# csiro-robotics/syropod_highlevel_controller

Hardware: AMD Instinct MI355X
Metric: control-cycles/sec (all legs IK-solved) (higher is better)
Workload: dtype f64

## Files before the change

### syropod_highlevel_controller_amd/csrc/shc_cycle.hpp

```cpp
#pragma once

#include "../../include/shc_batch.h"
#include "shc_leg.hpp"

namespace shc {

enum : int { WS_STARTING = 0, WS_MOVING = 1, WS_STOPPING = 2, WS_STOPPED = 3 };
enum : int { SS_SWING = 0, SS_STANCE = 1, SS_FORCE_STANCE = 2, SS_FORCE_STOP = 3 };
enum : int { PS_POSING = 0, PS_STOP_POSING = 1, PS_POSING_COMPLETE = 2 };
enum : int { PM_NONE = 0, PM_SWING = 1, PM_STANCE = 2, PM_STOP = 3 };

constexpr int LW_ACP = 1 << 2, LW_CFS = 1 << 3, LW_PM_SHIFT = 4, LW_NEG = 1 << 6, LW_IKFAIL = 1 << 7, LW_PHASE_SHIFT = 8,
              LW_PHASE_MASK = 0xFFFFF, LW_ZBV = 1 << 28, LW_ATT = 1 << 29, LW_ROTDEF = 1 << 30,
              LW_TARGROT = int(1u << 31);
constexpr int RW_LACP_SHIFT = 2, RW_LCFS_SHIFT = 6, RW_RTDA = 1 << 10, RW_APS_SHIFT = 11;

constexpr int kMaxAutoPosers = 8;
constexpr int kSwingTable = 64;
enum : unsigned { DIRTY_WALK_PLANE = 1, DIRTY_MANUAL = 2, DIRTY_SWING_ORG = 4, DIRTY_STANCE_ORG = 8,
                  DIRTY_TARG_DIR = 16,
                  DIRTY_LAST = DIRTY_TARG_DIR };
enum : unsigned { RT_MANUAL_LIVE = 1, RT_TOUCHDOWN = 2, RT_EXTERNAL = 4, RT_MANUAL_LEGS = 8, RT_EFFORT_LIVE = 16, RT_SKIP_MARKED = 32, RT_POSE_MARKED = 64 };

enum : unsigned { F_MANUAL = 1, F_AUTO = 2, F_INCL = 4, F_IMU = 8, F_ADM = 16, F_TIPF = 32, F_ODOM = 64, F_DYN = 1u << 31,
                  F_ROT = 1u << 30,
                  F_ROUGH = 1u << 29,
                  F_TALIGN = 1u << 28,
                  F_MLEGS = 1u << 27,
                  F_TERRAIN = F_ROUGH | F_TALIGN | F_MLEGS };
template <int NJ, unsigned F>
constexpr bool rot_enabled() { return (F & F_ROT) != 0 && (NJ > 3 || (F & F_MLEGS) != 0); }

struct CycleParams {
  double dt;
  int32_t period, swing_period, stance_period, stance_end, swing_start, swing_end, stance_start;
  int32_t remap_old_period;
  int32_t swing_iterations;
  int32_t stance_iterations;
  double swing_delta_t;
  double inv_dt;
  double dt_over_swing_dt;
  double stance_dt;
  double stride_scale;
  double swing_height, swing_width, body_clearance;
  double swing_progress_scaler;
  int32_t swing_c_count;
  int32_t swing_c_valid;
  int32_t velocity_input_mode;
  int32_t manual_posing, auto_posing, inclination_posing, imu_posing, admittance_control, dynamic_stiffness, use_joint_effort;
  int32_t clamp_joint_positions, clamp_joint_velocities, force_normal_touchdown;
  int32_t tip_force;
  int32_t debug_skip;
  int32_t odometry;
  int32_t gravity_aligned;
  int32_t rough_terrain;
  int32_t tip_align;
  int32_t gravity_target;
  int32_t joint_control;
  double step_depth;
  double target_dir[3];
  double max_translation[3], max_rotation[3], max_translation_velocity, max_rotation_velocity;
  double pid_p, pid_i, pid_d;
  double adm_m00, adm_m01, adm_m10, adm_m11, adm_g0, adm_g1;
  double force_gain, virtual_stiffness, swing_stiffness_scaler, load_stiffness_scaler;
  double pose_force_gain, pose_swing_height;
  int32_t n_auto_posers, pose_phase_length, pose_sync, auto_pose_reference_leg;
  alignas(16) int32_t ap_start[kMaxAutoPosers];
  int32_t ap_end[kMaxAutoPosers];
  double ap_amp[kMaxAutoPosers][7];
};

template <int L, int NJ>
struct alignas(16) SharedConsts {
  LegConst<NJ> leg[L];
  alignas(16) double limit[9][4];
  double swing_c[kSwingTable];
  alignas(16) CycleParams P;
};

template <int NJ>
struct Fields {
  static constexpr int NJE = (NJ + 1) & ~1;
  static constexpr int Q = 0, QD = NJ, TIP = 2 * NJ, TVEL = TIP + 3, SORG = TVEL + 3, SVEL = SORG + 3, TORG = SVEL + 3,
                       DFLT = TORG + 3, TARG = DFLT + 3, STRD = TARG + 3,
                       CORE_END = STRD + 3,
                       ADM = CORE_END, ADM_END = ADM + 2,
                       TF = ADM_END, TF_END = TF + 4,
                       FORCE_IN = TF_END, EFFORT_IN = FORCE_IN + 4,
                       POSER_TIP = EFFORT_IN + NJE, MODEL_TIP = POSER_TIP + 4, ADM_DELTA = MODEL_TIP + 4,
                       ORG_DIR = ADM_DELTA + 4, CUR_DIR = ORG_DIR + 3,
                       TARG_DIR = CUR_DIR + 3,
                       DES_TIP = TARG_DIR + 4, DES_DIR = DES_TIP + 4,
                       SEQ_ORG = DES_DIR + 4, SEQ_DIR = SEQ_ORG + 4, SEQ_Q0 = SEQ_DIR + 4,
                       STEP_PLANE = SEQ_Q0 + NJE,
                       MEAS_Q = STEP_PLANE + 4, COUNT = MEAS_Q + NJE;
  static_assert(CORE_END % 2 == 0 && SORG % 2 == 0 && COUNT % 2 == 0, "field groups must align to 16-byte planes");
};
SHC_HD int64_t leg_field_index(int f, int64_t slot, int64_t n_slots) { return (int64_t(f >> 1) * n_slots + slot) * 2 + (f & 1); }
struct RobotFields {
  static constexpr int VLIN = 0, VANG = 2, PLANE = 3, PNORM = 6, PLANE_PREV = 9, PNORM_PREV = 12, OWPP = 15, VIN = 22, WIN = 24,
                       CORE_END = 25;
  static constexpr int MPOSE = 25, TVI = 32, RVI = 35, MANUAL_END = 38;
  static constexpr int ABSE = 38, VERR = 41, GYRO = 44, IMU_END = 47;
  static constexpr int IMUQ = 47, IMUQ_END = 51;
  static constexpr int APREV = 51, APREV_END = 55;
  static constexpr int CPOSE = 55, CPOSE_END = 62;
  static constexpr int WPP = 62, WPP_END = 69;
  static constexpr int ODOM = 69, ODOM_END = 73;
  static constexpr int INCL = 73, INCL_END = 75;
  static constexpr int TALIGN = 75, OTALIGN = 82, COUNT = 89;
  static constexpr int I_WORD = 0, I_APOSER = 1, I_POSE_PHASE = 2, I_RESET_MODE = 3, I_COUNT = 4;
};

struct ExtFields {
  static constexpr int T_POSE = 0, T_TRANSFORM = 7, T_CLEARANCE = 14, T_FLAGS = 15,
                       D_POSE = 16, D_TRANSFORM = 23, D_FLAGS = 30,
                       P_POSE = 32, P_TRANSFORM = 39, P_CLEARANCE = 46, P_FLAGS = 47, COUNT = 48;
};

enum : int { LS_WALKING = 0, LS_MANUAL = 1, LS_WALKING_TO_MANUAL = -1, LS_MANUAL_TO_WALKING = -2 };
struct ManualRobot {
  int32_t leg_state[SHC_MAX_LEGS];
  int32_t manual_leg_count, primary_leg, secondary_leg;
  int32_t skip_cycle;
  double primary_velocity[3], secondary_velocity[3];
  double primary_position[3], secondary_position[3];
};

struct DevState {
  double *legd;
  int32_t *legi;
  double *robd;
  int32_t *robi;
  int64_t n_slots, n_rob_pad, n_robots;
  double *ext;
  ManualRobot *manual;
  const double *span;
};

struct SpanTable {
  static constexpr int kPlanes = 14;
  static constexpr int kStride = 2 + 2 * kPlanes;
};
SHC_HD double set_precision3(double v) { return round_to_int(v * 1000.0) / 1000.0; }
SHC_HD double stance_span_change_y(const double *table, int leg, double default_shift_z) {
  const double *t = table + leg * SpanTable::kStride;
  const int n = int(t[0]);
  const double target = set_precision3(default_shift_z);
  int lower = -1, upper = -1;
  for (int k = 0; k < n; ++k) {
    const double h = t[2 + 2 * k];
    if (h > target && (upper < 0 || h < t[2 + 2 * upper])) upper = k;
    if (h <= target && (lower < 0 || h > t[2 + 2 * lower])) lower = k;
  }
  if (lower < 0 || upper < 0) return 0.0;
  const double uh = set_precision3(t[2 + 2 * upper]), lh = set_precision3(t[2 + 2 * lower]);
  const double i = (target - lh) / (uh - lh);
  const double radius = t[3 + 2 * lower] * (1.0 - i) + t[3 + 2 * upper] * i;
  return radius * t[1];
}

#if defined(__HIPCC__)

template <int L, int NJ, unsigned F>
constexpr bool phase_fences() {
#if defined(SHC_FENCE)
  return true;
#else
  constexpr bool exact = (F & (0x80000000u  | 0x40000000u )) == 0;
  constexpr bool octo_tipf = L == 8 && NJ == 5 && (F & 32u ) != 0 && (F & 16u ) == 0;
  return exact && ((NJ == 4 && (L == 4 || L == 8)) || octo_tipf);
#endif
}
#define SHC_PHASE_FENCE() do { if constexpr (phase_fences<L, NJ, F>()) __builtin_amdgcn_sched_barrier(0); } while (0)
#if defined(SHC_RES2_TIMING) && !defined(SHC_RES2_BUSY_ONLY)
__shared__ long long shc_ticks_lds[64];
__shared__ long long shc_acc_lds[64];
#define SHC_TICK(i) do { __builtin_amdgcn_sched_barrier(0); if (blockIdx.x == 1 && (threadIdx.x == 0 || threadIdx.x == 128)) shc_ticks_lds[(threadIdx.x >> 7) * 32 + (i)] = __builtin_readcyclecounter(); __builtin_amdgcn_sched_barrier(0); } while (0)
#else
#define SHC_TICK(i) do {} while (0)
#endif
#ifdef SHC_ABLATE
#define SHC_DBG(P) ((P).debug_skip)
#else
#define SHC_DBG(P) 0
#endif
__device__ __forceinline__ int uni(int v) { return __builtin_amdgcn_readfirstlane(v); }

template <unsigned F>
struct Feat {
  __device__ __forceinline__ static bool manual(const CycleParams &P) { return (F & F_DYN) ? P.manual_posing != 0 : (F & F_MANUAL) != 0; }
  __device__ __forceinline__ static bool autop(const CycleParams &P) { return (F & F_DYN) ? P.auto_posing != 0 : (F & F_AUTO) != 0; }
  __device__ __forceinline__ static bool incl(const CycleParams &P) { return (F & F_DYN) ? P.inclination_posing != 0 : (F & F_INCL) != 0; }
  __device__ __forceinline__ static bool imu(const CycleParams &P) { return (F & F_DYN) ? P.imu_posing != 0 : (F & F_IMU) != 0; }
  __device__ __forceinline__ static bool adm(const CycleParams &P) { return (F & F_DYN) ? P.admittance_control != 0 : (F & F_ADM) != 0; }
  __device__ __forceinline__ static bool tipf(const CycleParams &P) { return (F & F_DYN) ? P.tip_force != 0 : (F & F_TIPF) != 0; }
  __device__ __forceinline__ static bool odom(const CycleParams &P) { return (F & F_DYN) ? P.odometry != 0 : (F & F_ODOM) != 0; }
};

template <int L>
struct Group {
  int base;
  __device__ __forceinline__ int get(int v, int j) const { return __shfl(v, base + j, 64); }
  __device__ __forceinline__ double get(double v, int j) const { return __shfl(v, base + j, 64); }
  __device__ __forceinline__ double sum(double v) const {
    double s = 0.0;
#pragma unroll
    for (int j = 0; j < L; ++j) s += get(v, j);
    return s;
  }
};

template <int RPW>
struct RobTile {
  double *d;
  int32_t *i;
  int grp;
  __device__ __forceinline__ double get(int f) const { return d[f * RPW + grp]; }
  __device__ __forceinline__ V3 get3(int f) const { return V3{d[f * RPW + grp], d[(f + 1) * RPW + grp], d[(f + 2) * RPW + grp]}; }
  __device__ __forceinline__ Quat getq(int f) const {
    return Quat{d[f * RPW + grp], d[(f + 1) * RPW + grp], d[(f + 2) * RPW + grp], d[(f + 3) * RPW + grp]};
  }
  __device__ __forceinline__ Pose getpose(int f) const { return Pose{get3(f), getq(f + 3)}; }
  __device__ __forceinline__ void put(int f, double v) const { d[f * RPW + grp] = v; }
  __device__ __forceinline__ void put3(int f, V3 v) const {
    d[f * RPW + grp] = v.x;
    d[(f + 1) * RPW + grp] = v.y;
    d[(f + 2) * RPW + grp] = v.z;
  }
  __device__ __forceinline__ void putq(int f, Quat q) const {
    d[f * RPW + grp] = q.w;
    d[(f + 1) * RPW + grp] = q.x;
    d[(f + 2) * RPW + grp] = q.y;
    d[(f + 3) * RPW + grp] = q.z;
  }
  __device__ __forceinline__ void putpose(int f, const Pose &p) const {
    put3(f, p.p);
    putq(f + 3, p.r);
  }
  __device__ __forceinline__ int geti(int f) const { return i[f * RPW + grp]; }
  __device__ __forceinline__ void puti(int f, int v) const { i[f * RPW + grp] = v; }
};

template <int NJ>
struct LegRegs {
  static constexpr bool kKeepJacobian = NJ <= 3;
  double q[NJ], qd[NJ];
  double sn[NJ], cs[NJ];
  V3 lin[NJ], pe;
  V3 tip, tvel, targ, strd;
  double adm0, adm1;
  double stiff;
  V3 tf, tipx;
  V3 org_dir, cur_dir, targ_dir;
  int word;
};

enum : int { PK_SORG = 0, PK_SVEL = 3, PK_TORG = 6, PK_DFLT = 9, PK_COUNT = 12 };
#ifndef SHC_PARK_REGS
struct Park {
  double *d;
  int lane;
  __device__ __forceinline__ V3 get3(int f) const { return V3{d[f * 64 + lane], d[(f + 1) * 64 + lane], d[(f + 2) * 64 + lane]}; }
  __device__ __forceinline__ void put3(int f, V3 v) const {
    d[f * 64 + lane] = v.x;
    d[(f + 1) * 64 + lane] = v.y;
    d[(f + 2) * 64 + lane] = v.z;
  }
  __device__ __forceinline__ double at(int k) const { return d[k * 64 + lane]; }
  __device__ __forceinline__ void set(int k, double v) const { d[k * 64 + lane] = v; }
};
#else
struct Park {
  double *d;
  int lane;
  mutable double r[12];
  __device__ __forceinline__ V3 get3(int f) const { return V3{r[f], r[f + 1], r[f + 2]}; }
  __device__ __forceinline__ void put3(int f, V3 v) const { r[f] = v.x, r[f + 1] = v.y, r[f + 2] = v.z; }
  __device__ __forceinline__ double at(int k) const { return r[k]; }
  __device__ __forceinline__ void set(int k, double v) const { r[k] = v; }
};
#endif

__device__ __forceinline__ V3 external_default(const double *ext, int64_t ns, uint32_t slot, V3 terrain_following) {
  if (ext == nullptr) return terrain_following;
  const double2 *X = reinterpret_cast<const double2 *>(ext);
  if ((int(X[(ExtFields::D_FLAGS / 2) * ns + slot].x) & 1) == 0) return terrain_following;
  double v[14];
#pragma unroll
  for (int k = 0; k < 7; ++k) {
    const double2 d = X[(ExtFields::D_POSE / 2 + k) * ns + slot];
    v[2 * k] = d.x, v[2 * k + 1] = d.y;
  }
  return V3{v[0], v[1], v[2]} + rotate(Quat{v[3], v[4], v[5], v[6]}, -V3{v[7], v[8], v[9]});
}

struct LegOut {
  V3 poser_tip, model_tip, adm_delta;
};

__device__ __forceinline__ double swing_progress_of(int word, const CycleParams &P) {
  int pm = (word >> LW_PM_SHIFT) & 3;
  if (pm != PM_SWING) return -1.0;
  int phase = (word >> LW_PHASE_SHIFT) & LW_PHASE_MASK;
  return clampd(double(phase - P.swing_start + 1) / double(P.swing_end - P.swing_start), 0.0, 1.0);
}

__device__ __forceinline__ int bearing_bracket(double y, double x) {
  if (x == 0.0 && y == 0.0) return 0;
  constexpr double kC = 0.99996192306417128874, kS = 0.0087265354983739347;
  double xr = kC * x - kS * y, yr = kS * x + kC * y;
  double ax = fabs(xr), ay = fabs(yr);
  bool upper = yr > 0.0 || (yr == 0.0 && xr > 0.0);
  if (upper) return xr > 0.0 ? (ay < ax ? 0 : 1) : (ay > ax ? 2 : 3);
  return xr < 0.0 ? (ay < ax ? 4 : 5) : (ay > ax ? 6 : 7);
}

template <int NJ>
struct LegInPlanes {
  const double *legd;
  int64_t ns;
  uint32_t slot;
  __device__ __forceinline__ V3 force() const {
    const double2 f01 = reinterpret_cast<const double2 *>(legd)[(Fields<NJ>::FORCE_IN / 2) * ns + slot];
    const double2 f2_ = reinterpret_cast<const double2 *>(legd)[(Fields<NJ>::FORCE_IN / 2 + 1) * ns + slot];
    return V3{f01.x, f01.y, f2_.x};
  }
  __device__ __forceinline__ void effort(double (&e)[NJ]) const {
#pragma unroll
    for (int i = 0; i < NJ; i += 2) {
      const double2 e2 = reinterpret_cast<const double2 *>(legd)[((Fields<NJ>::EFFORT_IN + i) / 2) * ns + slot];
      e[i] = e2.x;
      if (i + 1 < NJ) e[i + 1] = e2.y;
    }
  }
};
struct NoHook {
  __device__ __forceinline__ void operator()() const {}
};

struct UniFlags {
  int clamp_joint_velocities, clamp_joint_positions, swing_c_count;
  int velocity_input_mode, force_normal_touchdown;
};
__device__ __forceinline__ UniFlags load_uni_flags(const CycleParams &P) {
  const int c = P.clamp_joint_velocities, d = P.clamp_joint_positions, e = P.swing_c_count;
  const int f = P.velocity_input_mode, h = P.force_normal_touchdown;
  return UniFlags{uni(c), uni(d), uni(e), uni(f), uni(h)};
}

struct FrontToBack {
  V3 desired_dir;
  bool rot_def;
  int my_leg_state;
  bool plane_prev_changed;
  bool pose_only;
  V3 odom_vel;
  bool odom_run;
  bool joint_moved;
  V3 held_pe, held_dir;
  bool planes_in_sync = false;
  UniFlags uf;
  int limit_bracket = -1;
  double limit_value[4] = {0.0, 0.0, 0.0, 0.0};
};

struct OdomCache {
  double ha = 0.0, sh = 0.0, ch = 1.0;
  bool valid = false;
};
__device__ __forceinline__ void odometry_advance(double &ox, double &oy, double &ow, double &oz, const CycleParams &P, double vx, double vy, double vw,
                                                 OdomCache *cache = nullptr) {
  double sh, ch;
  const double ha = 0.5 * (vw * P.dt);
  if (cache != nullptr && cache->valid && __all(ha == cache->ha)) {
    sh = cache->sh, ch = cache->ch;
  } else {
    if (__all(fabs(ha) <= 0.5)) sincos_joint<false>(ha, &sh, &ch);
    else sincos_joint(ha, &sh, &ch);
    if (cache != nullptr) cache->ha = ha, cache->sh = sh, cache->ch = ch, cache->valid = true;
  }
  {
#pragma clang fp contract(off)
    const double a = vx * P.dt, b = vy * P.dt;
    double ux = -(oz * b), uy = oz * a;
    ux = ux + ux;
    uy = uy + uy;
    const double nx = ox + fma(-oz, uy, fma(ux, ow, a)), ny = oy + fma(oz, ux, fma(uy, ow, b));
    const double nw = fma(ow, ch, -(oz * sh)), nz = fma(ow, sh, oz * ch);
    ox = nx, oy = ny, ow = nw, oz = nz;
  }
}
template <int RPW>
__device__ __forceinline__ void odometry_step(const RobTile<RPW> &rb, const CycleParams &P, double vx, double vy, double vw, OdomCache *cache = nullptr) {
  using R = RobotFields;
  double ox = rb.get(R::ODOM), oy = rb.get(R::ODOM + 1), ow = rb.get(R::ODOM + 2), oz = rb.get(R::ODOM + 3);
  odometry_advance(ox, oy, ow, oz, P, vx, vy, vw, cache);
  rb.put(R::ODOM, ox);
  rb.put(R::ODOM + 1, oy);
  rb.put(R::ODOM + 2, ow);
  rb.put(R::ODOM + 3, oz);
}

template <int L, int NJ>
__device__ __forceinline__ double walk_plane_control_input(const int own_word, const SharedConsts<L, NJ> &C, const CycleParams &P, const Group<L> g,
                                                           const int swing_c_count_u) {
  double c = 0.0;
  bool sel = false;
  if (swing_c_count_u > 0) {
    const int it_own = min(max(((own_word >> LW_PHASE_SHIFT) & LW_PHASE_MASK) - P.swing_start, 0), P.swing_c_count - 1);
    const bool ok_own = ((own_word >> LW_PM_SHIFT) & 3) == PM_SWING && it_own < P.swing_c_valid;
    const unsigned legs_ok = unsigned((__ballot(ok_own) >> g.base) & ((1ull << L) - 1));
    sel = legs_ok != 0;
    const int last = sel ? 31 - __clz(int(legs_ok)) : 0;
    int it_sel = g.get(it_own, last);
    it_sel = sel ? it_sel : 0;
    if (__any(sel)) c = sel ? C.swing_c[it_sel] : 0.0;
  } else {
    double c_own = -1.0;
    const double sp = swing_progress_of(own_word, P) * P.swing_progress_scaler;
    if (sp >= 0 && sp <= 1.0) c_own = smooth_step(sp);
#pragma unroll
    for (int j = 0; j < L; ++j) {
      const double cj = g.get(c_own, j);
      if (cj >= 0.0) {
        c = cj;
        sel = true;
      }
    }
  }
  return sel ? c : -1.0;
}

template <int L, int NJ>
__device__ __forceinline__ double walk_plane_control_candidate(const int own_word, const SharedConsts<L, NJ> &C, const CycleParams &P, const int swing_c_count_u) {
  if (swing_c_count_u > 0) {
    const int it_own = min(max(((own_word >> LW_PHASE_SHIFT) & LW_PHASE_MASK) - P.swing_start, 0), P.swing_c_count - 1);
    const bool ok_own = ((own_word >> LW_PM_SHIFT) & 3) == PM_SWING && it_own < P.swing_c_valid;
    const double c = C.swing_c[it_own];
    return ok_own ? c : -1.0;
  }
  const double sp = swing_progress_of(own_word, P) * P.swing_progress_scaler;
  return (sp >= 0 && sp <= 1.0) ? smooth_step(sp) : -1.0;
}

template <int L>
__device__ __forceinline__ V3 quat_to_euler_zyx_grouped(Quat q, const Group<L> g, const int leg) {
  static_assert(L >= 3, "three lanes per robot");
  double tx = 2.0 * q.x, ty = 2.0 * q.y, tz = 2.0 * q.z;
  double twx = tx * q.w, twy = ty * q.w, twz = tz * q.w;
  double txx = tx * q.x, txy = ty * q.x, txz = tz * q.x;
  double tyy = ty * q.y, tyz = tz * q.y, tzz = tz * q.z;
  double m00 = 1.0 - (tyy + tzz), m01 = txy - twz, m02 = txz + twy;
  double m10 = txy + twz, m11 = 1.0 - (txx + tzz), m12 = tyz - twx;
  double m20 = txz - twy, m21 = tyz + twx, m22 = 1.0 - (txx + tyy);
  const double c2 = sqrt(m22 * m22 + m21 * m21);
  const bool neg = m10 < 0.0 || (m10 == 0.0 && __builtin_signbit(m10) && __builtin_signbit(m00));
  const bool second = leg == 1;
  const double t = atan2(second ? -m20 : m10, second ? (neg ? -c2 : c2) : m00);
  double r0 = g.get(t, 0), r1 = g.get(t, 1);
  if (__builtin_expect(__any((r0 < 0.0) != neg), 0)) r1 = atan2(-m20, r0 < 0.0 ? -c2 : c2);
  if (r0 < 0.0) r0 += kPi;
  double s1, c1;
  sincos_joint(r0, &s1, &c1);
  double r2 = atan2(s1 * m02 - c1 * m12, c1 * m11 - s1 * m01);
  if (fabs(r1) > kPi / 2 || fabs(r2) > kPi / 2) {
    r0 -= kPi;
    if (r1 > kPi / 2.0) r1 = -r1 + kPi;
    else if (r1 < kPi / 2.0) r1 = -r1 - kPi;
    if (r2 > kPi / 2.0) r2 -= kPi;
    else if (r2 < kPi / 2.0) r2 += kPi;
  }
  return V3{r2, r1, r0};
}
template <int L>
__device__ __forceinline__ Quat euler_to_quat_zyx_grouped(V3 e, const Group<L> g, const int leg) {
  static_assert(L >= 3, "three lanes per robot");
  double sn, cs;
  sincos_joint(0.5 * (leg == 0 ? e.x : (leg == 1 ? e.y : e.z)), &sn, &cs);
  const double sx = g.get(sn, 0), cx = g.get(cs, 0), sy = g.get(sn, 1), cy = g.get(cs, 1), sz = g.get(sn, 2), cz = g.get(cs, 2);
  Quat qx{cx, sx, 0, 0}, qy{cy, 0, sy, 0}, qz{cz, 0, 0, sz};
// ... 1139 lines not shown
```

### syropod_highlevel_controller_amd/csrc/shc_cycle_inst.hip

```cpp
#include "shc_cycle_kernel.hpp"
#include "shc_cycle_select.hpp"

#if !defined(SHC_INST_L) || !defined(SHC_INST_NJ) || !defined(SHC_INST_PART)
#error "compile with -DSHC_INST_L=<legs> -DSHC_INST_NJ=<joints> -DSHC_INST_PART=<0|1>"
#endif

#include <cstdio>
#include <cstdlib>
#include <mutex>
#include <set>
#include <tuple>

namespace shc {

static void note_kernel(const char *form, int legs, int joints, unsigned features) {
  static const char *path = std::getenv("SHC_KERNEL_LOG");
  if (!path) return;
  static std::mutex mu;
  static std::set<std::tuple<const char *, unsigned>> seen;
  std::lock_guard<std::mutex> lock(mu);
  if (!seen.insert({form, features}).second) return;
  if (FILE *f = std::fopen(path, "a")) {
    std::fprintf(f, "%s %d %d %u\n", form, legs, joints, features);
    std::fclose(f);
  }
}

template <int L, int NJ, unsigned F>
static void launch_cycle(const CycleLaunch &a) {
  constexpr int RPW = 64 / L;
  constexpr size_t wave_bytes = size_t(RobotFields::COUNT * RPW + PK_COUNT * 64 + (RobotFields::I_COUNT * RPW + 1) / 2) * 8;
#if SHC_INST_PART == 1
  if (a.fit) {
    a.fit->supported = has_resident(F) ? 1 : 0;
    a.fit->batch = has_batch(F) ? 1 : 0;
    a.fit->two_wave = has_two_wave(F) ? 1 : 0;
    a.fit->blocks_per_cu = 0;
    if constexpr (has_resident(F)) {
      int blocks = 0;
      if (hipOccupancyMaxActiveBlocksPerMultiprocessor(&blocks, shc_resident_kernel<L, NJ, F>, 64, wave_bytes) != hipSuccess) blocks = 0;
      a.fit->blocks_per_cu = blocks;
    }
  } else if (a.resident->batch_cycles != 0) {
    if constexpr (has_batch(F)) {
      note_kernel("batch", L, NJ, F);
      shc_batch_kernel<L, NJ, F><<<dim3(a.grid), dim3(a.block), wave_bytes * (a.block / 64), a.stream>>>(a.st, (const SharedConsts<L, NJ> *)a.consts, *a.resident, a.rt_flags);
    }
  } else if (a.block == 256) {
    if constexpr (has_two_wave(F)) {
      note_kernel("resident2", L, NJ, F);
      shc_resident2_kernel<L, NJ, F><<<dim3(a.grid), dim3(256), 2 * wave_bytes + sizeof(Resident2Lds<L, NJ>), a.stream>>>(
          a.st, (const SharedConsts<L, NJ> *)a.consts, *a.resident, a.rt_flags);
    }
  } else {
    if constexpr (has_resident(F)) {
      note_kernel("resident", L, NJ, F);
      shc_resident_kernel<L, NJ, F><<<dim3(a.grid), dim3(64), wave_bytes, a.stream>>>(a.st, (const SharedConsts<L, NJ> *)a.consts, *a.resident, a.rt_flags);
    }
  }
#else
  if constexpr (has_half_kernels(F)) {
    const int64_t waves = int64_t(a.grid) * (a.block / 64);
    if (a.half_steps >= 0 && (a.half_steps > 0 || waves >= 2048)) {
      note_kernel("half", L, NJ, F);
      for (int c = 0; c < a.n_cycles; ++c) {
        shc_cycle_half_kernel<L, NJ, F, ROLE_FRONT><<<dim3(a.grid), dim3(a.block), wave_bytes * (a.block / 64), a.stream>>>(
            a.st, (const SharedConsts<L, NJ> *)a.consts, a.rt_flags, a.wave0);
        shc_cycle_half_kernel<L, NJ, F, ROLE_BACK><<<dim3(a.grid), dim3(a.block), wave_bytes * (a.block / 64), a.stream>>>(
            a.st, (const SharedConsts<L, NJ> *)a.consts, a.rt_flags, a.wave0);
      }
      return;
    }
  }
  note_kernel("cycle", L, NJ, F);
  shc_cycle_kernel<L, NJ, F><<<dim3(a.grid), dim3(a.block), wave_bytes * (a.block / 64), a.stream>>>(a.st, (const SharedConsts<L, NJ> *)a.consts, a.n_cycles,
                                                                                              a.rt_flags, a.wave0);
#endif
}

template <int L, int NJ, unsigned... Fs>
static bool launch_selected(const CycleLaunch &a, FeatureList<Fs...>) {
  const unsigned f = select_features(L, NJ, *a.cp, a.rt_flags, a.generic);
  return ((f == Fs && (launch_cycle<L, NJ, Fs>(a), true)) || ...);
}

#define SHC_CAT3(a, b, c) a##b##_##c
#define SHC_LAUNCHER_NAME(L_, NJ_) SHC_CAT3(shc_launch_cycle_, L_, NJ_)
#define SHC_LOOP_LAUNCHER_NAME(L_, NJ_) SHC_CAT3(shc_launch_loop_, L_, NJ_)
#if SHC_INST_PART == 1
bool SHC_LOOP_LAUNCHER_NAME(SHC_INST_L, SHC_INST_NJ)(const CycleLaunch &a) { return launch_selected<SHC_INST_L, SHC_INST_NJ>(a, KernelTable<SHC_INST_L, SHC_INST_NJ>{}); }
#else
bool SHC_LOOP_LAUNCHER_NAME(SHC_INST_L, SHC_INST_NJ)(const CycleLaunch &a);
bool SHC_LAUNCHER_NAME(SHC_INST_L, SHC_INST_NJ)(const CycleLaunch &a) {
  if (a.fit || a.resident) return SHC_LOOP_LAUNCHER_NAME(SHC_INST_L, SHC_INST_NJ)(a);
  return launch_selected<SHC_INST_L, SHC_INST_NJ>(a, KernelTable<SHC_INST_L, SHC_INST_NJ>{});
}
#endif

}
```

### syropod_highlevel_controller_amd/csrc/shc_cycle_kernel.hpp

```cpp
#pragma once

#include "shc_cycle.hpp"
#include "shc_cycle_launch.hpp"

#include <hip/hip_runtime.h>

namespace shc {

#ifndef SHC_WAVES_PER_SIMD
#define SHC_WAVES_PER_SIMD 2
#endif
#ifndef SHC_ROT_WAVES_PER_SIMD
#define SHC_ROT_WAVES_PER_SIMD 1
#endif
#ifndef SHC_TERRAIN_WAVES_PER_SIMD
#define SHC_TERRAIN_WAVES_PER_SIMD 2
#endif

struct LegPlanes {
  double2 *base;
  int64_t ns;
  uint32_t slot;
  typedef double v2d __attribute__((ext_vector_type(2)));
  __device__ __forceinline__ double2 load(int plane) const { return (base + plane * ns)[slot]; }
  __device__ __forceinline__ void store(int plane, double2 v) const {
    v2d w = {v.x, v.y};
    __builtin_nontemporal_store(w, reinterpret_cast<v2d *>(base + plane * ns + slot));
  }
};

template <int NJ>
struct LegLoad {
  double flat[Fields<NJ>::CORE_END];
  double2 adm, tf0, tf1, stiff, rot0, rot1, rot2, rot3, rot4;
  int word;
};
enum : int { ROLE_ALL = 0, ROLE_FRONT = 1, ROLE_BACK = 2 };
template <int NJ, unsigned F, int ROLE = ROLE_ALL>
__device__ __forceinline__ void load_leg_issue(LegLoad<NJ> &ll, const DevState &st, const CycleParams &P, uint32_t slot) {
  using FD = Fields<NJ>;
  using FT = Feat<F>;
  const LegPlanes ld{reinterpret_cast<double2 *>(st.legd), st.n_slots, slot};
#pragma unroll
  for (int p = 0; p < FD::CORE_END / 2; ++p) {
    if ((ROLE == ROLE_FRONT && p < NJ) || (ROLE == ROLE_BACK && p >= NJ)) {
      ll.flat[2 * p] = ll.flat[2 * p + 1] = 0.0;
      continue;
    }
    double2 v = ld.load(p);
    ll.flat[2 * p] = v.x;
    ll.flat[2 * p + 1] = v.y;
  }
  ll.word = ROLE == ROLE_BACK ? 0 : st.legi[slot];
  ll.adm = ll.tf0 = ll.tf1 = ll.stiff = ll.rot0 = ll.rot1 = ll.rot2 = ll.rot3 = ll.rot4 = double2{0.0, 0.0};
  if (rot_enabled<NJ, F>() && ROLE != ROLE_BACK) {
    ll.rot0 = ld.load(FD::ORG_DIR / 2);
    ll.rot1 = ld.load(FD::ORG_DIR / 2 + 1);
    ll.rot2 = ld.load(FD::ORG_DIR / 2 + 2);
    ll.rot3 = ld.load(FD::ORG_DIR / 2 + 3);
    ll.rot4 = ld.load(FD::ORG_DIR / 2 + 4);
  }
  if (FT::adm(P)) {
    if (ROLE != ROLE_FRONT) ll.adm = ld.load(FD::ADM / 2);
    if (ROLE != ROLE_BACK && P.dynamic_stiffness) ll.stiff = ld.load(FD::ADM_DELTA / 2 + 1);
  }
  if (FT::tipf(P) && ROLE != ROLE_FRONT) {
    ll.tf0 = ld.load(FD::TF / 2);
    ll.tf1 = ld.load(FD::TF / 2 + 1);
  }
}
template <int NJ, int ROLE = ROLE_ALL>
__device__ __forceinline__ void load_leg_finish(LegRegs<NJ> &s, const Park &pk, const LegLoad<NJ> &ll) {
  using FD = Fields<NJ>;
  const double(&flat)[FD::CORE_END] = ll.flat;
  s.word = ll.word;
  static_assert(FD::SVEL == FD::SORG + 3 && FD::TORG == FD::SORG + 6 && FD::DFLT == FD::SORG + 9, "park layout");
  if (ROLE != ROLE_BACK) {
#pragma unroll
    for (int k = 0; k < PK_COUNT; ++k) pk.set(k, flat[FD::SORG + k]);
  }
  s.tip = V3{flat[FD::TIP + 0], flat[FD::TIP + 1], flat[FD::TIP + 2]};
  s.targ = V3{flat[FD::TARG + 0], flat[FD::TARG + 1], flat[FD::TARG + 2]};
  s.strd = V3{flat[FD::STRD + 0], flat[FD::STRD + 1], flat[FD::STRD + 2]};
  s.tvel = V3{flat[FD::TVEL + 0], flat[FD::TVEL + 1], flat[FD::TVEL + 2]};
#pragma unroll
  for (int i = 0; i < NJ; ++i) {
    s.q[i] = flat[FD::Q + i];
    s.qd[i] = flat[FD::QD + i];
  }
  s.adm0 = ll.adm.x;
  s.adm1 = ll.adm.y;
  s.stiff = ll.stiff.y;
  s.tf = V3{ll.tf0.x, ll.tf0.y, ll.tf1.x};
  s.org_dir = V3{ll.rot0.x, ll.rot0.y, ll.rot1.x};
  s.cur_dir = V3{ll.rot1.y, ll.rot2.x, ll.rot2.y};
  s.targ_dir = V3{ll.rot3.x, ll.rot3.y, ll.rot4.x};
}

template <int NJ, unsigned F, int ROLE = ROLE_ALL, bool SPLIT = false>
__device__ __forceinline__ void store_leg(const LegRegs<NJ> &s, const LegOut &out, const Park &pk, const DevState &st, const CycleParams &P,
                                          uint32_t slot, unsigned dirty) {
  using FD = Fields<NJ>;
  using FT = Feat<F>;
  const LegPlanes ld{reinterpret_cast<double2 *>(st.legd), st.n_slots, slot};
  double flat[FD::CORE_END];
#pragma unroll
  for (int i = 0; i < NJ; ++i) {
    flat[FD::Q + i] = s.q[i];
    flat[FD::QD + i] = s.qd[i];
  }
  flat[FD::TIP] = s.tip.x, flat[FD::TIP + 1] = s.tip.y, flat[FD::TIP + 2] = s.tip.z;
  flat[FD::TVEL] = s.tvel.x, flat[FD::TVEL + 1] = s.tvel.y, flat[FD::TVEL + 2] = s.tvel.z;
#pragma unroll
  for (int k = 0; k < PK_COUNT; ++k) flat[FD::SORG + k] = ROLE == ROLE_BACK ? 0.0 : pk.at(k);
  flat[FD::TARG] = s.targ.x, flat[FD::TARG + 1] = s.targ.y, flat[FD::TARG + 2] = s.targ.z;
  flat[FD::STRD] = s.strd.x, flat[FD::STRD + 1] = s.strd.y, flat[FD::STRD + 2] = s.strd.z;
  static_assert(FD::SORG % 2 == 0 && FD::TORG % 2 == 0 && FD::TARG % 2 == 0, "park groups must cover whole planes");
#pragma unroll
  for (int p = 0; p < FD::CORE_END / 2; ++p) {
    const bool swing_org = 2 * p >= FD::SORG && 2 * p < FD::TORG, stance_org = 2 * p >= FD::TORG && 2 * p < FD::TARG;
    if (swing_org && !(dirty & DIRTY_SWING_ORG)) continue;
    if (stance_org && !(dirty & DIRTY_STANCE_ORG)) continue;
    if ((ROLE == ROLE_FRONT && p < NJ) || (ROLE == ROLE_BACK && p >= NJ)) continue;
    ld.store(p, double2{flat[2 * p], flat[2 * p + 1]});
  }
  if (FT::adm(P) && ROLE != ROLE_FRONT && !(SPLIT && ROLE == ROLE_BACK)) {
    ld.store(FD::ADM / 2, double2{s.adm0, s.adm1});
    ld.store(FD::ADM_DELTA / 2, double2{out.adm_delta.x, out.adm_delta.y});
    ld.store(FD::ADM_DELTA / 2 + 1, double2{out.adm_delta.z, s.stiff});
  }
  if (SPLIT && ROLE == ROLE_FRONT && FT::adm(P) && P.dynamic_stiffness) st.legd[leg_field_index(FD::ADM_DELTA + 3, slot, st.n_slots)] = s.stiff;
  if (FT::tipf(P) && ROLE != ROLE_FRONT) {
    ld.store(FD::TF / 2, double2{s.tf.x, s.tf.y});
    ld.store(FD::TF / 2 + 1, double2{s.tf.z, 0.0});
  }
  if (FT::autop(P) && !FT::imu(P) && ROLE != ROLE_BACK) {
    ld.store(FD::POSER_TIP / 2, double2{out.poser_tip.x, out.poser_tip.y});
    ld.store(FD::POSER_TIP / 2 + 1, double2{out.poser_tip.z, 0.0});
  }
  if (rot_enabled<NJ, F>() && ROLE != ROLE_BACK) {
    static_assert(FD::ORG_DIR % 2 == 0 && FD::CUR_DIR == FD::ORG_DIR + 3 && FD::TARG_DIR == FD::ORG_DIR + 6, "tip direction planes");
    ld.store(FD::ORG_DIR / 2, double2{s.org_dir.x, s.org_dir.y});
    ld.store(FD::ORG_DIR / 2 + 1, double2{s.org_dir.z, s.cur_dir.x});
    ld.store(FD::ORG_DIR / 2 + 2, double2{s.cur_dir.y, s.cur_dir.z});
    if (dirty & DIRTY_TARG_DIR) {
      ld.store(FD::ORG_DIR / 2 + 3, double2{s.targ_dir.x, s.targ_dir.y});
      ld.store(FD::ORG_DIR / 2 + 4, double2{s.targ_dir.z, 0.0});
    }
  }
  if (ROLE != ROLE_BACK) st.legi[slot] = s.word;
}

template <int NJ>
__device__ __forceinline__ void store_admittance_early(const LegRegs<NJ> &s, const LegOut &out, const DevState &st, uint32_t slot) {
  using FD = Fields<NJ>;
  const LegPlanes ld{reinterpret_cast<double2 *>(st.legd), st.n_slots, slot};
  ld.store(FD::ADM / 2, double2{s.adm0, s.adm1});
  ld.store(FD::ADM_DELTA / 2, double2{out.adm_delta.x, out.adm_delta.y});
  st.legd[leg_field_index(FD::ADM_DELTA + 2, slot, st.n_slots)] = out.adm_delta.z;
}

template <int RPW, int F0, int F1>
__device__ __forceinline__ void load_rob_fields(double (&reg)[((F1 - F0) * RPW + 63) / 64], const double *gtile, int lane) {
  constexpr int total = (F1 - F0) * RPW;
  constexpr int iters = (total + 63) / 64;
#pragma unroll
  for (int it = 0; it < iters; ++it) {
    int idx = it * 64 + lane;
    reg[it] = idx < total ? gtile[F0 * RPW + idx] : 0.0;
  }
}
template <int RPW, int F0, int F1>
__device__ __forceinline__ void put_rob_fields(const double (&reg)[((F1 - F0) * RPW + 63) / 64], double *tile, int lane) {
  constexpr int total = (F1 - F0) * RPW;
  constexpr int iters = (total + 63) / 64;
#pragma unroll
  for (int it = 0; it < iters; ++it) {
    int idx = it * 64 + lane;
    if (idx < total) tile[F0 * RPW + idx] = reg[it];
  }
}
template <int RPW, int F0, int F1>
__device__ __forceinline__ void store_rob_fields(const double *tile, double *gtile, int lane) {
  constexpr int total = (F1 - F0) * RPW;
  constexpr int iters = (total + 63) / 64;
#pragma unroll
  for (int it = 0; it < iters; ++it) {
    int idx = it * 64 + lane;
    if (idx < total) gtile[F0 * RPW + idx] = tile[F0 * RPW + idx];
  }
}

typedef unsigned long long u64;
__device__ __forceinline__ u64 ld_agent(const u64 *p) { return __hip_atomic_load(p, __ATOMIC_RELAXED, __HIP_MEMORY_SCOPE_AGENT); }
__device__ __forceinline__ void st_agent(u64 *p, u64 v) { __hip_atomic_store(p, v, __ATOMIC_RELAXED, __HIP_MEMORY_SCOPE_AGENT); }
__device__ __forceinline__ u64 ld_sys(const u64 *p) { return __hip_atomic_load(p, __ATOMIC_RELAXED, __HIP_MEMORY_SCOPE_SYSTEM); }
__device__ __forceinline__ void st_sys(u64 *p, u64 v) { __hip_atomic_store(p, v, __ATOMIC_RELAXED, __HIP_MEMORY_SCOPE_SYSTEM); }
__device__ __forceinline__ double ld_agent_f64(const double *p) { return __longlong_as_double((long long)ld_agent(reinterpret_cast<const u64 *>(p))); }
__device__ __forceinline__ u64 uni64(u64 v) {
  const unsigned lo = __builtin_amdgcn_readfirstlane(unsigned(v)), hi = __builtin_amdgcn_readfirstlane(unsigned(v >> 32));
  return (u64(hi) << 32) | lo;
}

template <int NJ>
struct LegInRing {
  const double *force_ptr = nullptr, *effort_ptr = nullptr;
  int64_t force_pair = 0, effort_pair = 0;
  bool effort_prefetched = false;
  double effort_now[NJ] = {};
  bool coherent = true;
  bool force_prefetched = false;
  double force_now[3] = {};
  __device__ __forceinline__ double ld(const double *p) const { return coherent ? ld_agent_f64(p) : *p; }
  __device__ __forceinline__ void prefetch_effort() {
#pragma unroll
    for (int i = 0; i < NJ; ++i) effort_now[i] = ld(effort_ptr + int64_t(i / 2) * effort_pair + (i & 1));
    effort_prefetched = true;
  }
  __device__ __forceinline__ void prefetch_force() {
    force_now[0] = ld(force_ptr), force_now[1] = ld(force_ptr + 1), force_now[2] = ld(force_ptr + force_pair);
    force_prefetched = true;
  }
  __device__ __forceinline__ V3 force() const {
    if (force_prefetched) return V3{force_now[0], force_now[1], force_now[2]};
    return V3{ld(force_ptr), ld(force_ptr + 1), ld(force_ptr + force_pair)};
  }
  __device__ __forceinline__ void effort(double (&e)[NJ]) const {
    if (effort_prefetched) {
#pragma unroll
      for (int i = 0; i < NJ; ++i) e[i] = effort_now[i];
      return;
    }
#pragma unroll
    for (int i = 0; i < NJ; ++i) e[i] = ld(effort_ptr + int64_t(i / 2) * effort_pair + (i & 1));
  }
};
__device__ __forceinline__ const double *bound_array(const ResidentArgs &A, int set, int which) {
  const double *const *row = set == 0 ? A.bound[0] : (set == 1 ? A.bound[1] : (set == 2 ? A.bound[2] : A.bound[3]));
  return which == BND_LIN ? row[BND_LIN] : which == BND_ANG ? row[BND_ANG] : which == BND_IMUQ ? row[BND_IMUQ] : which == BND_IMUW ? row[BND_IMUW]
       : which == BND_FORCE ? row[BND_FORCE] : row[BND_EFFORT];
}
template <int L, int NJ>
__device__ __forceinline__ LegInRing<NJ> leg_inputs_in_force(const ResidentArgs &A, const double *legd, const int src_force, const int src_effort, const int64_t ns,
                                                             const uint32_t slot, const int64_t robot, const int leg, const int64_t row = 0) {
  using FD = Fields<NJ>;
  LegInRing<NJ> in;
  const double *fplanes = src_force < 0 ? legd + int64_t(FD::FORCE_IN / 2) * ns * 2 : A.force + int64_t(src_force) * 2 * ns * 2;
  const double *eplanes = src_effort < 0 ? legd + int64_t(FD::EFFORT_IN / 2) * ns * 2 : A.effort + int64_t(src_effort) * (FD::NJE / 2) * ns * 2;
  in.force_ptr = fplanes + int64_t(slot) * 2, in.force_pair = ns * 2;
  in.effort_ptr = eplanes + int64_t(slot) * 2, in.effort_pair = ns * 2;
  if (src_force <= -2) in.force_ptr = bound_array(A, -2 - src_force, BND_FORCE) + row * A.kstride[BND_FORCE] + (robot * L + leg) * 3, in.force_pair = 2;
  if (src_effort <= -2) in.effort_ptr = bound_array(A, -2 - src_effort, BND_EFFORT) + row * A.kstride[BND_EFFORT] + (robot * L + leg) * NJ, in.effort_pair = 2;
  return in;
}

struct ResidentHeld {
  int src_force = -1, src_effort = -1;
  unsigned seen = 0;
  unsigned cycles = 0;
  bool fault = false;
};

template <int RPW, int NF>
__device__ __forceinline__ void ring_to_tile(const double *rec, double *tile_at, int lane) {
  constexpr int total = NF * RPW;
#pragma unroll
  for (int it = 0; it * 64 < total; ++it) {
    const int i = it * 64 + lane;
    if (i < total) tile_at[i] = ld_agent_f64(rec + i);
  }
}

enum : int { ROBOT_NONE = 0, ROBOT_VEL = 1, ROBOT_POSE = 2, ROBOT_ALL = 3 };
template <int RPW, int ROBOT, bool LEG>
__device__ __forceinline__ void resident_take_inputs(const ResidentArgs &A, const unsigned c, const u64 h0, const u64 h1, const int64_t wave, const int lane,
                                                     double *tile, int32_t *tile_i, unsigned &dirty, ResidentHeld &held, const int64_t n_robots, const int64_t row = 0) {
  using R = RobotFields;
  if (h0 != u64(c) + 1) return;
  const unsigned mask = unsigned(h1) & 0x7fffu;
  held.seen |= mask;
  if (unsigned(h1) & kResidentDirect) {
    const int set = int((h1 >> 16) & 3);
    if (ROBOT != ROBOT_NONE) {
      if ((ROBOT & ROBOT_VEL) && (mask & (1u << RG_VEL))) {
        static_assert(R::WIN == R::VIN + 2, "velocity inputs are contiguous in the tile");
        const double *lin = bound_array(A, set, BND_LIN) + row * A.kstride[BND_LIN], *ang = bound_array(A, set, BND_ANG) + row * A.kstride[BND_ANG];
        const int field = lane / RPW, r = lane - field * RPW;
        const int64_t rob = wave * RPW + r;
        if (lane < 3 * RPW && rob < n_robots) tile[(R::VIN + field) * RPW + r] = field < 2 ? ld_agent_f64(lin + rob * 2 + field) : ld_agent_f64(ang + rob);
      }
      if ((ROBOT & ROBOT_POSE) && (mask & (1u << RG_IMU))) {
        const int64_t rob = wave * RPW + lane;
        if (lane < RPW && rob < n_robots) {
          const double *q = bound_array(A, set, BND_IMUQ) + row * A.kstride[BND_IMUQ] + rob * 4, *w = bound_array(A, set, BND_IMUW) + row * A.kstride[BND_IMUW] + rob * 3;
          const Quat qn = normalized(Quat{ld_agent_f64(q), ld_agent_f64(q + 1), ld_agent_f64(q + 2), ld_agent_f64(q + 3)});
          tile[(R::IMUQ + 0) * RPW + lane] = qn.w, tile[(R::IMUQ + 1) * RPW + lane] = qn.x, tile[(R::IMUQ + 2) * RPW + lane] = qn.y, tile[(R::IMUQ + 3) * RPW + lane] = qn.z;
#pragma unroll
          for (int k = 0; k < 3; ++k) tile[(R::GYRO + k) * RPW + lane] = ld_agent_f64(w + k);
        }
      }
      __builtin_amdgcn_fence(__ATOMIC_RELEASE, "wavefront");
      __builtin_amdgcn_wave_barrier();
    }
    if (LEG) {
      if (mask & (1u << RG_FORCE)) held.src_force = -2 - set;
      if (mask & (1u << RG_EFFORT)) held.src_effort = -2 - set;
    }
    return;
// ... 338 lines not shown
          st_agent(&A.ctl->pad[1], m);
          asm volatile("s_waitcnt vmcnt(0)" ::: "memory");
          st_agent(&A.ctl->pad[2], 1ull);
          st_sys(&A.host->exited, (fault || gave_up) ? u64(RESIDENT_EXIT_FAULT) : why);
        }
      }
      if ((++iter & 1023) == 0 && lane == 0) st_sys(&A.host->heartbeat, iter);
    }
    if (leave) break;
    __builtin_amdgcn_s_sleep(1);
  }
}

template <int L, int NJ, unsigned F, bool RES, int HALF = ROLE_ALL, bool BATCH = false>
__device__ __forceinline__ void cycle_wave(const DevState &st, const SharedConsts<L, NJ> *gc, int n_cycles, unsigned rt_flags, const int64_t wave,
                                           const ResidentArgs *ra) {
  static_assert(HALF == ROLE_ALL || (!RES && (F & (F_DYN | F_TERRAIN | F_MLEGS | F_AUTO)) == 0), "half-step launches: feature-exact kernels without auto posing / terrain paths");
  using R = RobotFields;
  using FT = Feat<F>;
  constexpr int RPW = 64 / L;
  __shared__ SharedConsts<L, NJ> C;
  extern __shared__ double wave_lds[];
  constexpr int kWaveDoubles = R::COUNT * RPW + PK_COUNT * 64 + (R::I_COUNT * RPW + 1) / 2;
  SHC_TICK(0);
  const bool manual_live = (rt_flags & RT_MANUAL_LIVE) != 0;
  const bool touchdown_detection = (rt_flags & RT_TOUCHDOWN) != 0;
  const int lane = threadIdx.x & 63;
  const int wib = threadIdx.x >> 6;
  const int64_t rob0 = wave * RPW;
  const int64_t left = st.n_robots - rob0;
  const int robots_here = left < RPW ? (left < 0 ? 0 : int(left)) : RPW;
  int grp = lane / L;
  const int leg = lane - grp * L;
  const bool live = grp < robots_here;
  if (grp >= robots_here) grp = robots_here > 0 ? robots_here - 1 : 0;
  const uint32_t slot = uint32_t(wave * 64 + grp * L + leg);
  double *const my_lds = wave_lds + wib * kWaveDoubles;
  Park pk{my_lds + R::COUNT * RPW, lane};
  LegRegs<NJ> s;
  const CycleParams &GP = gc->P;
  double *tile = my_lds;
  int32_t *tile_i = reinterpret_cast<int32_t *>(my_lds + R::COUNT * RPW + PK_COUNT * 64);
  double *gtile = st.robd + wave * (R::COUNT * RPW);
  int32_t *gtile_i = st.robi + wave * (R::I_COUNT * RPW);
  LegLoad<NJ> ll;
  double th[NJ];
  const bool any_robot = robots_here > 0;
  double2 hand[4] = {double2{0.0, 0.0}, double2{0.0, 0.0}, double2{0.0, 0.0}, double2{0.0, 0.0}};
  double hpose[7] = {0.0, 0.0, 0.0, 1.0, 0.0, 0.0, 0.0};
  double2 qpl[(NJ + 1) / 2];
  int word_back = 0;
  if (any_robot) {
#pragma unroll
    for (int k = 0; k < NJ; ++k) th[k] = gc->leg[leg].link_th[k];
    load_leg_issue<NJ, F, HALF>(ll, st, GP, slot);
    if constexpr (HALF == ROLE_FRONT) {
#pragma unroll
      for (int p = 0; p < (NJ + 1) / 2; ++p) qpl[p] = reinterpret_cast<const double2 *>(st.legd)[p * st.n_slots + slot];
    }
    if constexpr (HALF == ROLE_BACK) {
      word_back = st.legi[slot];
      using FDh = Fields<NJ>;
      static_assert(FDh::TIP % 2 == 0 && FDh::CUR_DIR == FDh::ORG_DIR + 3 && FDh::ORG_DIR % 2 == 0, "plane layout of the walker tip / tip direction");
      const double2 *planes = reinterpret_cast<const double2 *>(st.legd);
      hand[0] = planes[(FDh::TIP / 2) * st.n_slots + slot];
      hand[1] = planes[(FDh::TIP / 2 + 1) * st.n_slots + slot];
      hand[2] = planes[(FDh::ORG_DIR / 2 + 1) * st.n_slots + slot];
      hand[3] = planes[(FDh::ORG_DIR / 2 + 2) * st.n_slots + slot];
#pragma unroll
      for (int k = 0; k < 7; ++k) hpose[k] = gtile[(R::CPOSE + k) * RPW + grp];
    }
  }
  using SC = SharedConsts<L, NJ>;
  static_assert(sizeof(SC) % 16 == 0 && (offsetof(SC, P) + offsetof(CycleParams, ap_start)) % 16 == 0, "const block is copied in 16-byte words");
  constexpr int n16_all = sizeof(SC) / 16;
  constexpr int n16_core = (offsetof(SC, P) + offsetof(CycleParams, ap_start)) / 16;
  const int n16 = FT::autop(GP) ? n16_all : n16_core;
  constexpr int citers = (n16_all + 63) / 64;
  double2 creg[citers];
  {
    const double2 *src = reinterpret_cast<const double2 *>(gc);
    const int nt = blockDim.x;
#pragma unroll
    for (int it = 0; it < citers; ++it) {
      int i = it * nt + threadIdx.x;
      creg[it] = i < n16 ? src[i] : double2{0.0, 0.0};
    }
  }
  double t_core[(R::CORE_END * RPW + 63) / 64], t_man[((R::MANUAL_END - R::MPOSE) * RPW + 63) / 64],
      t_imu[((R::IMU_END - R::ABSE) * RPW + 63) / 64], t_imuq[((R::IMUQ_END - R::IMUQ) * RPW + 63) / 64],
      t_aprev[((R::APREV_END - R::APREV) * RPW + 63) / 64], t_align[((R::COUNT - R::TALIGN) * RPW + 63) / 64], t_odom[((R::ODOM_END - R::ODOM) * RPW + 63) / 64],
      t_cpose[((R::CPOSE_END - R::CPOSE) * RPW + 63) / 64], t_incl[((R::INCL_END - R::INCL) * RPW + 63) / 64];
  const bool skip_marked = (F & F_MLEGS) != 0 && (rt_flags & RT_SKIP_MARKED) != 0 && (rt_flags & RT_MANUAL_LEGS) != 0;
  const bool pose_marked = (F & F_MLEGS) != 0 && (rt_flags & RT_POSE_MARKED) != 0 && (rt_flags & RT_MANUAL_LEGS) != 0;
  constexpr int int_iters = (R::I_COUNT * RPW + 63) / 64;
  int32_t t_int[int_iters];
  if (any_robot && HALF == ROLE_BACK) {
#pragma unroll
    for (int k = 0; k < NJ; ++k) sincos_joint(th[k] + ll.flat[Fields<NJ>::Q + k], &s.sn[k], &s.cs[k]);
    load_leg_finish<NJ, HALF>(s, pk, ll);
    s.word = word_back;
  }
  if (any_robot && HALF != ROLE_BACK) {
    load_rob_fields<RPW, 0, R::CORE_END>(t_core, gtile, lane);
    if (FT::manual(GP) && manual_live) load_rob_fields<RPW, R::MPOSE, R::MANUAL_END>(t_man, gtile, lane);
    if (FT::imu(GP)) load_rob_fields<RPW, R::ABSE, R::IMU_END>(t_imu, gtile, lane);
    if (FT::imu(GP) || FT::incl(GP) || FT::autop(GP)) load_rob_fields<RPW, R::IMUQ, R::IMUQ_END>(t_imuq, gtile, lane);
    if (FT::incl(GP) && FT::autop(GP)) load_rob_fields<RPW, R::APREV, R::APREV_END>(t_aprev, gtile, lane);
    if (FT::odom(GP)) load_rob_fields<RPW, R::ODOM, R::ODOM_END>(t_odom, gtile, lane);
    if (skip_marked || pose_marked) load_rob_fields<RPW, R::CPOSE, R::CPOSE_END>(t_cpose, gtile, lane);
    if (pose_marked && FT::incl(GP)) load_rob_fields<RPW, R::INCL, R::INCL_END>(t_incl, gtile, lane);
    if ((F & F_TALIGN) != 0 && GP.tip_align) load_rob_fields<RPW, R::TALIGN, R::COUNT>(t_align, gtile, lane);
#pragma unroll
    for (int it = 0; it < int_iters; ++it) t_int[it] = it * 64 + lane < R::I_COUNT * RPW ? gtile_i[it * 64 + lane] : 0;
#pragma unroll
    for (int k = 0; k < NJ; ++k) {
      double qk = ll.flat[Fields<NJ>::Q + k];
      if constexpr (HALF == ROLE_FRONT) qk = (k & 1) ? qpl[k / 2].y : qpl[k / 2].x;
      sincos_joint(th[k] + qk, &s.sn[k], &s.cs[k]);
    }
    load_leg_finish<NJ, HALF>(s, pk, ll);
  }
  {
    double2 *dst = reinterpret_cast<double2 *>(&C);
    const int nt = blockDim.x;
#pragma unroll
    for (int it = 0; it < citers; ++it) {
      int i = it * nt + threadIdx.x;
      if (i < n16) dst[i] = creg[it];
    }
  }
  if (any_robot && HALF != ROLE_BACK) {
    put_rob_fields<RPW, 0, R::CORE_END>(t_core, tile, lane);
    if (FT::manual(GP) && manual_live) put_rob_fields<RPW, R::MPOSE, R::MANUAL_END>(t_man, tile, lane);
    if (FT::imu(GP)) put_rob_fields<RPW, R::ABSE, R::IMU_END>(t_imu, tile, lane);
    if (FT::imu(GP) || FT::incl(GP) || FT::autop(GP)) put_rob_fields<RPW, R::IMUQ, R::IMUQ_END>(t_imuq, tile, lane);
    if (FT::incl(GP) && FT::autop(GP)) put_rob_fields<RPW, R::APREV, R::APREV_END>(t_aprev, tile, lane);
    if (FT::odom(GP)) put_rob_fields<RPW, R::ODOM, R::ODOM_END>(t_odom, tile, lane);
    if (skip_marked || pose_marked) put_rob_fields<RPW, R::CPOSE, R::CPOSE_END>(t_cpose, tile, lane);
    if (pose_marked && FT::incl(GP)) put_rob_fields<RPW, R::INCL, R::INCL_END>(t_incl, tile, lane);
    if ((F & F_TALIGN) != 0 && GP.tip_align) put_rob_fields<RPW, R::TALIGN, R::COUNT>(t_align, tile, lane);
#pragma unroll
    for (int it = 0; it < int_iters; ++it)
      if (it * 64 + lane < R::I_COUNT * RPW) tile_i[it * 64 + lane] = t_int[it];
  }
  SHC_TICK(18);
  __syncthreads();
  SHC_TICK(19);
  if (robots_here == 0) return;
  const CycleParams &P = C.P;
  Group<L> g{grp * L};
  RobTile<RPW> rb{tile, tile_i, grp};
  s.tipx = V3{1, 0, 0};
  constexpr bool rot_on = rot_enabled<NJ, F>();
  if (FT::adm(P) || LegRegs<NJ>::kKeepJacobian || rot_on) {
    Chain<NJ> ch;
    chain_from_sincos<NJ>(C.leg[leg], s.sn, s.cs, ch);
    if (LegRegs<NJ>::kKeepJacobian) {
      jacobian_columns<NJ>(ch, s.lin);
      s.pe = ch.pe;
    }
    if (FT::adm(P) || rot_on) s.tipx = base_rotate(C.leg[leg], ch.xe);
  }
  LegOut out;
  SHC_TICK(1);
  unsigned dirty = 0;
  double *const ext = ((F & F_ROUGH) != 0 && (rt_flags & RT_EXTERNAL) != 0) ? st.ext : nullptr;
  const ManualRobot *const mr = ((F & F_MLEGS) != 0 && (rt_flags & RT_MANUAL_LEGS) != 0 && any_robot) ? st.manual + (rob0 + grp) : nullptr;
  const bool marked = mr != nullptr && mr->skip_cycle != 0;
  const bool skip = (skip_marked && marked) || (pose_marked && !marked);
  const bool pose_only = pose_marked && marked;
  ResidentHeld held;
  if constexpr (RES) {
    resident_loop<L, NJ, F, BATCH>(*ra, st, s, out, C, rb, pk, g, leg, slot, lane, wave, live, tile, tile_i, dirty, manual_live, held, touchdown_detection, ext);
  } else if constexpr (HALF == ROLE_FRONT) {
    FrontToBack fb;
    fb.planes_in_sync = false;
    fb.limit_bracket = -1;
    fb.uf = load_uni_flags(C.P);
    fb.pose_only = false;
    cycle_front<L, NJ, F, (F & F_ADM) == 0>(s, out, C, rb, pk, g, leg, st.legd, st.n_slots, slot, dirty, manual_live, touchdown_detection, ext, mr,
                                            LegInPlanes<NJ>{st.legd, st.n_slots, slot}, fb);
  } else if constexpr (HALF == ROLE_BACK) {
    FrontToBack fb;
    fb.uf = load_uni_flags(C.P);
    fb.pose_only = false;
    fb.joint_moved = false;
    fb.my_leg_state = 0;
    fb.rot_def = (s.word & LW_ROTDEF) != 0;
    {
      const Pose bp{V3{hpose[0], hpose[1], hpose[2]}, Quat{hpose[3], hpose[4], hpose[5], hpose[6]}};
      out.poser_tip = inverse_transform_vector(bp, V3{hand[0].x, hand[0].y, hand[1].x});
      fb.desired_dir = V3{1, 0, 0};
      if (fb.rot_def) fb.desired_dir = rotate(inverse(bp.r), V3{hand[2].y, hand[3].x, hand[3].y});
    }
    out.adm_delta = V3{0.0, 0.0, 0.0};
    if (FT::adm(P)) {
      cycle_admittance<NJ>(s, out, P, LegInPlanes<NJ>{st.legd, st.n_slots, slot});
      if (live && !skip) store_admittance_early<NJ>(s, out, st, slot);
    }
    cycle_back<L, NJ, F>(s, out, C, leg, st.legd, st.n_slots, slot, mr, LegInPlanes<NJ>{st.legd, st.n_slots, slot}, fb);
  } else if (!skip) {
    for (int c = 0; c < n_cycles; ++c)
      cycle<L, NJ, F>(s, out, C, rb, pk, g, leg, st.legd, st.n_slots, slot, dirty, manual_live, touchdown_detection, ext, mr,
                      LegInPlanes<NJ>{st.legd, st.n_slots, slot}, NoHook(), (F & F_ROUGH) != 0 ? st.span : nullptr, pose_only);
    if ((F & F_MLEGS) != 0 && pose_only && FT::autop(P) && !FT::imu(P)) {
      const double2 *planes = reinterpret_cast<const double2 *>(st.legd);
      const double2 a = planes[(Fields<NJ>::POSER_TIP / 2) * st.n_slots + slot], b = planes[(Fields<NJ>::POSER_TIP / 2 + 1) * st.n_slots + slot];
      out.poser_tip = V3{a.x, a.y, b.x};
    }
  }
  {
    unsigned d = 0;
#pragma unroll
    for (unsigned b = 1; b <= DIRTY_LAST; b <<= 1)
      if (__any((dirty & b) != 0)) d |= b;
    dirty = d;
  }
  if (live && !skip) store_leg<NJ, F, HALF, HALF != ROLE_ALL>(s, out, pk, st, P, slot, dirty);
  if constexpr (HALF == ROLE_BACK) {
    if (live) st.legi[slot] = s.word;
    return;
  }
  SHC_TICK(13);
  __builtin_amdgcn_wave_barrier();
  store_rob_fields<RPW, 0, R::PLANE>(tile, gtile, lane);
  if (dirty & DIRTY_WALK_PLANE) store_rob_fields<RPW, R::PLANE, R::VIN>(tile, gtile, lane);
  if (FT::manual(P) && manual_live && (dirty & DIRTY_MANUAL)) store_rob_fields<RPW, R::MPOSE, R::MANUAL_END>(tile, gtile, lane);
  if (FT::imu(P)) store_rob_fields<RPW, R::ABSE, R::GYRO>(tile, gtile, lane);
  if (FT::incl(P) && FT::autop(P)) store_rob_fields<RPW, R::APREV, R::APREV_END>(tile, gtile, lane);
  if ((F & F_MLEGS) != 0 && FT::incl(P) && pose_marked) store_rob_fields<RPW, R::INCL, R::INCL_END>(tile, gtile, lane);
  store_rob_fields<RPW, R::CPOSE, R::CPOSE_END>(tile, gtile, lane);
  if (FT::odom(P)) store_rob_fields<RPW, R::ODOM, R::ODOM_END>(tile, gtile, lane);
  if ((F & F_TALIGN) != 0 && P.tip_align) store_rob_fields<RPW, R::TALIGN, R::COUNT>(tile, gtile, lane);
  static_assert((R::I_POSE_PHASE + 1) * RPW <= 64, "the written-back int fields (word, poser latches, pose phase) fit one wave-wide store");
  if (lane < (R::I_POSE_PHASE + 1) * RPW) gtile_i[lane] = tile_i[lane];
  if constexpr (RES) resident_epilogue<L, NJ, F>(*ra, st, slot, lane, live, tile, tile_i, gtile, gtile_i, held);
  SHC_TICK(14);
}

template <int L, int NJ, unsigned F>
__global__ void __launch_bounds__(256, (F & F_ROT) ? SHC_ROT_WAVES_PER_SIMD : ((F & F_DYN) && (F & F_TERRAIN)) ? SHC_TERRAIN_WAVES_PER_SIMD : SHC_WAVES_PER_SIMD) shc_cycle_kernel(DevState st, const SharedConsts<L, NJ> *gc, int n_cycles,
                                                                                             unsigned rt_flags, int64_t wave0) {
  cycle_wave<L, NJ, F, false>(st, gc, n_cycles, rt_flags, wave0 + ((int64_t(blockIdx.x) * blockDim.x + threadIdx.x) >> 6), nullptr);
}

template <int L, int NJ, unsigned F, int HALF>
__global__ void __launch_bounds__(256, 2) shc_cycle_half_kernel(DevState st, const SharedConsts<L, NJ> *gc, unsigned rt_flags, int64_t wave0) {
  cycle_wave<L, NJ, F, false, HALF>(st, gc, 1, rt_flags, wave0 + ((int64_t(blockIdx.x) * blockDim.x + threadIdx.x) >> 6), nullptr);
}

template <int L, int NJ, unsigned F>
__global__ void __launch_bounds__(64, (F & (F_ROT | F_ROUGH)) ? 1 : SHC_WAVES_PER_SIMD) shc_resident_kernel(DevState st, const SharedConsts<L, NJ> *gc, ResidentArgs ra, unsigned rt_flags) {
  if (blockIdx.x == 0) {
    resident_relay<PART_BOTH>(ra);
    return;
  }
  cycle_wave<L, NJ, F, true>(st, gc, 0, rt_flags, int64_t(blockIdx.x) - 1, &ra);
}

template <int L, int NJ, unsigned F>
__global__ void __launch_bounds__(256, (F & F_ROT) ? SHC_ROT_WAVES_PER_SIMD : SHC_WAVES_PER_SIMD) shc_batch_kernel(DevState st, const SharedConsts<L, NJ> *gc, ResidentArgs ra, unsigned rt_flags) {
  cycle_wave<L, NJ, F, true, ROLE_ALL, true>(st, gc, 0, rt_flags, ra.batch_wave0 + ((int64_t(blockIdx.x) * blockDim.x + threadIdx.x) >> 6), &ra);
}

enum : int { IT_REAL = 1, IT_BUBBLE = 2, IT_EXIT = 3 };
template <int RPW>
struct PoseWait {
  unsigned *flag_at;
  unsigned want;
  u64 ticks_per_ms;
  bool *fault;
  __device__ __forceinline__ bool give_up(unsigned &spins, u64 &t0) const {
    __builtin_amdgcn_s_sleep(1);
    if ((++spins & 4095u) == 0) {
      const u64 now = wall_clock64();
      if (t0 == 0) t0 = now;
      else if (now - t0 > 1000 * ticks_per_ms) {
        *fault = true;
        return true;
      }
    }
    return false;
  }
  __device__ __forceinline__ void operator()() const {
    volatile unsigned *flag = flag_at;
    unsigned spins = 0;
    u64 t0 = 0;
    while (*flag != want)
      if (give_up(spins, t0)) break;
    __builtin_amdgcn_fence(__ATOMIC_ACQUIRE, "workgroup");
  }
};
template <int L, int NJ>
struct Resident2Lds {
  double mailbox[2][2][13][64];
  double pose_c[2][2][64];
  unsigned pose_done[2];
  unsigned model_dirty[2], model_seen[2], model_fault[2];
  double stiff[2][64];
  int ikfail[2][64];
  unsigned long long ctrl[4][4];
};

template <int L, int NJ, unsigned F>
__global__ void __launch_bounds__(256, 1) shc_resident2_kernel(DevState st, const SharedConsts<L, NJ> *gc, ResidentArgs A, unsigned rt_flags) {
  using R = RobotFields;
  using FD = Fields<NJ>;
  using FT = Feat<F>;
  constexpr int RPW = 64 / L;
  if (blockIdx.x == 0) {
    if (threadIdx.x < 64) resident_relay<PART_GATE>(A);
    else if (threadIdx.x < 128) resident_relay<PART_DONE>(A);
    return;
  }
  __shared__ SharedConsts<L, NJ> C;
  extern __shared__ double wave_lds[];
  constexpr int kWaveDoubles = R::COUNT * RPW + PK_COUNT * 64 + (R::I_COUNT * RPW + 1) / 2;
  Resident2Lds<L, NJ> &X = *reinterpret_cast<Resident2Lds<L, NJ> *>(wave_lds + 2 * kWaveDoubles);
  const bool manual_live = (rt_flags & RT_MANUAL_LIVE) != 0;
  const int lane = threadIdx.x & 63;
  const int wib = __builtin_amdgcn_readfirstlane(threadIdx.x >> 6);
  const int pair = wib & 1;
  const bool walker = wib < 2, leader = wib == 2;
  const int64_t wave = (int64_t(blockIdx.x) - 1) * 2 + pair;
  const bool active = wave < A.n_waves;
  const int64_t rob0 = wave * RPW;
  const int64_t left = st.n_robots - rob0;
  const int robots_here = !active ? 0 : (left < RPW ? (left < 0 ? 0 : int(left)) : RPW);
  int grp = lane / L;
  const int leg = lane - grp * L;
  const bool live = grp < robots_here;
  if (grp >= robots_here) grp = robots_here > 0 ? robots_here - 1 : 0;
  const uint32_t slot = uint32_t((active ? wave : 0) * 64 + grp * L + leg);
  double *const my_lds = wave_lds + pair * kWaveDoubles;
  Park pk{my_lds + R::COUNT * RPW, lane};
  double *tile = my_lds;
  int32_t *tile_i = reinterpret_cast<int32_t *>(my_lds + R::COUNT * RPW + PK_COUNT * 64);
  double *gtile = st.robd + (active ? wave : 0) * (R::COUNT * RPW);
  int32_t *gtile_i = st.robi + (active ? wave : 0) * (R::I_COUNT * RPW);
  const CycleParams &GP = gc->P;
  LegRegs<NJ> s;
  {
    using SC = SharedConsts<L, NJ>;
    constexpr int n16_all = sizeof(SC) / 16;
    constexpr int n16_core = (offsetof(SC, P) + offsetof(CycleParams, ap_start)) / 16;
    const int n16 = FT::autop(GP) ? n16_all : n16_core;
    const double2 *src = reinterpret_cast<const double2 *>(gc);
    double2 *dst = reinterpret_cast<double2 *>(&C);
    for (int i = threadIdx.x; i < n16; i += 256) dst[i] = src[i];
  }
  LegLoad<NJ> ll;
  if (active) {
    if (walker) {
      load_leg_issue<NJ, F, ROLE_FRONT>(ll, st, GP, slot);
      for (int i = lane; i < R::COUNT * RPW; i += 64) tile[i] = gtile[i];
      for (int i = lane; i < R::I_COUNT * RPW; i += 64) tile_i[i] = gtile_i[i];
      load_leg_finish<NJ, ROLE_FRONT>(s, pk, ll);
    } else {
      load_leg_issue<NJ, F, ROLE_BACK>(ll, st, GP, slot);
      load_leg_finish<NJ, ROLE_BACK>(s, pk, ll);
    }
  }
  if (leader && lane == 0) {
    X.ctrl[0][0] = IT_BUBBLE;
    X.ctrl[0][1] = X.ctrl[0][2] = 0;
  }
  constexpr bool POSE_SPLIT = (F & (F_DYN | F_AUTO)) == 0;
  if (POSE_SPLIT && walker && lane == 0) X.pose_done[pair] = 0;
  __syncthreads();
  const CycleParams &P = C.P;
  Group<L> g{grp * L};
  RobTile<RPW> rb{tile, tile_i, grp};
  LegOut out;
  out.poser_tip = out.model_tip = out.adm_delta = V3{0, 0, 0};
  s.tipx = V3{1, 0, 0};
  if (active && !walker) {
#pragma unroll
    for (int k = 0; k < NJ; ++k) sincos_joint(C.leg[leg].link_th[k] + s.q[k], &s.sn[k], &s.cs[k]);
    if (FT::adm(P) || LegRegs<NJ>::kKeepJacobian) {
      Chain<NJ> ch;
      chain_from_sincos<NJ>(C.leg[leg], s.sn, s.cs, ch);
      if (LegRegs<NJ>::kKeepJacobian) {
        jacobian_columns<NJ>(ch, s.lin);
        s.pe = ch.pe;
      }
      if (FT::adm(P)) s.tipx = base_rotate(C.leg[leg], ch.xe);
    }
    s.word = 0;
  }
  unsigned dirty = 0;
  ResidentHeld held;
  const int swing_c_count_u = uni(P.swing_c_count);
  const auto publish_for_pose = [&](unsigned cycle, bool planes) {
    if (planes) {
      const V3 pp = rb.get3(R::PLANE_PREV), pn = rb.get3(R::PNORM_PREV);
#pragma unroll
      for (int par = 0; par < 2; ++par) {
        double *mb = &X.mailbox[pair][par][0][lane];
        mb[7 * 64] = pp.x, mb[8 * 64] = pp.y, mb[9 * 64] = pp.z, mb[10 * 64] = pn.x, mb[11 * 64] = pn.y, mb[12 * 64] = pn.z;
      }
    }
    X.pose_c[pair][cycle & 1][lane] = walk_plane_control_candidate<L, NJ>(s.word, C, P, swing_c_count_u);
  };
  if (POSE_SPLIT && walker && active) publish_for_pose(0, true);
  const int64_t ns = st.n_slots;
  const unsigned out_slot_bytes = unsigned(NJ * ns * 16);
  const __amdgpu_buffer_rsrc_t out_rsrc = __builtin_amdgcn_make_buffer_rsrc(A.out, 0, int(unsigned(A.depth) * out_slot_bytes), 0x00020000);
  const u64 emergency_ticks = 4 * A.idle_ticks + 2000 * A.ticks_per_ms;
  unsigned k = 0, c_front = 0, c_back = 0, oslot = 0;
  bool prev_real = false;
  u64 prev_h0 = 0, prev_h1 = 0;
  u64 gate_pref = leader ? ld_agent(&A.ctl->gate) : 0;
  u64 bubble_since = 0;
  FrontToBack fb{V3{1, 0, 0}, false, LS_WALKING};
  fb.uf = load_uni_flags(C.P);
  OdomCache odom_cache;
  Pose owpp_cache = pose_identity();
  if (POSE_SPLIT && active && !walker) owpp_cache = rb.getpose(R::OWPP);
  constexpr bool ODOM_REGS = NJ <= 3;
  constexpr bool ODOM_WALKER = NJ > 3 || (F & (F_ADM | F_IMU | F_INCL | F_AUTO | F_DYN)) != 0;
  double odom[4] = {0.0, 0.0, 1.0, 0.0};
  if (ODOM_REGS && FT::odom(P) && active && walker == ODOM_WALKER) {
#pragma unroll
    for (int i = 0; i < 4; ++i) odom[i] = rb.get(R::ODOM + i);
  }
#ifdef SHC_RES2_TIMING
  long long tm_busy = 0, tm_total0 = __builtin_readcyclecounter(), tm_real = 0;
#ifndef SHC_RES2_BUSY_ONLY
  if (threadIdx.x < 64) shc_acc_lds[threadIdx.x] = 0;
#endif
#endif
#ifdef SHC_RES2_TIMING
#define SHC_R2_ITER_BEGIN() const long long tm0 = __builtin_readcyclecounter(); SHC_TICK(19)
#ifndef SHC_RES2_BUSY_ONLY
#define SHC_R2_PHASES(THREAD, ...)                                                                                                  \
  if (kind == IT_REAL && prev_real && blockIdx.x == 1 && threadIdx.x == (THREAD)) {       \
    const int base = ((THREAD) >> 7) * 32;                                                                                         \
    const int order[] = {__VA_ARGS__};                                                                                             \
    for (int i = 1; i < int(sizeof(order) / sizeof(int)); ++i) shc_acc_lds[base + order[i]] += shc_ticks_lds[base + order[i]] - shc_ticks_lds[base + order[i - 1]]; \
  }
#else
#define SHC_R2_PHASES(THREAD, ...)
#endif
#define SHC_R2_ITER_END(THREAD, ...)                                                         \
  if (kind == IT_REAL && prev_real) tm_busy += __builtin_readcyclecounter() - tm0, ++tm_real; \
  SHC_R2_PHASES(THREAD, __VA_ARGS__)
#else
#define SHC_R2_ITER_BEGIN() do {} while (0)
#define SHC_R2_ITER_END(THREAD, ...) do {} while (0)
#endif
  LegInRing<NJ> in_at;
  int in_src_force = -1000, in_src_effort = -1000;
  if (walker) {
    for (;;) {
      SHC_R2_ITER_BEGIN();
      const int kind = __builtin_amdgcn_readfirstlane(int(X.ctrl[k & 3][0]));
      const u64 h0 = uni64(X.ctrl[k & 3][1]), h1 = uni64(X.ctrl[k & 3][2]);
      SHC_TICK(20);
      if (kind == IT_REAL && active) {
        resident_take_inputs<RPW, POSE_SPLIT ? ROBOT_VEL : ROBOT_ALL, false>(A, c_front, h0, h1, wave, lane, tile, tile_i, dirty, held, st.n_robots);
        SHC_TICK(21);
        const PoseWait<RPW> pose_wait{&X.pose_done[pair], c_front + 1, A.ticks_per_ms, &held.fault};
        cycle_front<L, NJ, F, false, LegInRing<NJ>, false, !POSE_SPLIT>(s, out, C, rb, pk, g, leg, st.legd, ns, slot, dirty, manual_live, false, nullptr, nullptr,
                                                                        LegInRing<NJ>{}, fb, nullptr, pose_wait);
#ifdef SHC_ABLATE
        if (!(P.debug_skip & 65536))
#endif
        if (POSE_SPLIT) publish_for_pose(c_front + 1, fb.plane_prev_changed);
        SHC_TICK(29);
        double *mb = &X.mailbox[pair][c_front & 1][0][lane];
        mb[0] = out.poser_tip.x, mb[64] = out.poser_tip.y, mb[128] = out.poser_tip.z;
        if constexpr (ODOM_WALKER) {
          if (FT::odom(P) && __any(fb.odom_run)) {
            if (fb.odom_run) {
              if constexpr (ODOM_REGS) odometry_advance(odom[0], odom[1], odom[2], odom[3], P, fb.odom_vel.x, fb.odom_vel.y, fb.odom_vel.z, &odom_cache);
              else odometry_step(rb, P, fb.odom_vel.x, fb.odom_vel.y, fb.odom_vel.z, &odom_cache);
            }
          }
        } else if (FT::odom(P)) {
          mb[192] = fb.odom_vel.x, mb[256] = fb.odom_vel.y, mb[320] = fb.odom_vel.z, mb[384] = fb.odom_run ? 1.0 : 0.0;
        }
        SHC_TICK(22);
      }
      SHC_TICK(23);
      if (kind == IT_EXIT) break;
      SHC_R2_ITER_END(0, 19, 20, 21, 2, 3, 4, 5, 6, 7, 16, 8, 17, 15, 29, 22, 23);
      if (kind == IT_REAL) ++c_front;
      prev_real = kind == IT_REAL;
      __syncthreads();
      ++k;
    }
  } else {
    for (;;) {
      SHC_R2_ITER_BEGIN();
      const int kind = __builtin_amdgcn_readfirstlane(int(X.ctrl[k & 3][0]));
      const u64 h0 = uni64(X.ctrl[k & 3][1]), h1 = uni64(X.ctrl[k & 3][2]);
      SHC_TICK(29);
      int nk = IT_EXIT;
      u64 nh0v = 0, nh1v = 0;
      if (leader && kind != IT_EXIT) {
        u64 gate;
        if (kind == IT_BUBBLE) {
          __builtin_amdgcn_s_sleep(2);
          gate = uni64(ld_agent(&A.ctl->gate));
        } else {
          gate = uni64(gate_pref);
        }
        const unsigned db = unsigned(gate), sp = unsigned(gate >> 32);
        const unsigned cn = c_front + (kind == IT_REAL ? 1u : 0u);
        nk = cn >= sp ? IT_EXIT : (cn < db ? IT_REAL : IT_BUBBLE);
        if (nk == IT_BUBBLE) {
          const u64 now = wall_clock64();
          if (bubble_since == 0) bubble_since = now;
          else if (now - bubble_since > emergency_ticks) nk = IT_EXIT, held.fault = true;
        } else {
          bubble_since = 0;
        }
        if (nk == IT_REAL) {
          const u64 *hp = reinterpret_cast<const u64 *>(A.headers + (cn & (kResidentHeaders - 1)));
          nh0v = ld_agent(hp);
          nh1v = ld_agent(hp + 1);
        }
        if (kind == IT_BUBBLE) gate_pref = gate;
        else gate_pref = ld_agent(&A.ctl->gate);
      }
      if (active) {
        SHC_TICK(24);
        if constexpr (POSE_SPLIT) if (kind == IT_REAL) {
          resident_take_inputs<RPW, ROBOT_POSE, false>(A, c_front, h0, h1, wave, lane, tile, tile_i, dirty, held, st.n_robots);
          SHC_TICK(30);
          double pose_c = -1.0;
#pragma unroll
          for (int j = 0; j < L; ++j) {
            const double cj = X.pose_c[pair][c_front & 1][g.base + j];
            pose_c = cj >= 0.0 ? cj : pose_c;
          }
          int lw[L] = {};
          const double *mb = &X.mailbox[pair][c_front & 1][0][lane];
          const V3 plane_prev{mb[7 * 64], mb[8 * 64], mb[9 * 64]}, pnorm_prev{mb[10 * 64], mb[11 * 64], mb[12 * 64]};
          int rword_unused = 0;
          Pose ap = pose_identity(), la = pose_identity();
#ifdef SHC_ABLATE
          if (!(P.debug_skip & 2048))
#endif
          (void)cycle_pose<L, NJ, F, true>(s, C, P, C.leg[leg], rb, g, leg, lw, rword_unused, 0, dirty, manual_live, ap, la, plane_prev, pnorm_prev, fb.uf.swing_c_count, 0,
                                           &owpp_cache, &pose_c);
          __builtin_amdgcn_fence(__ATOMIC_RELEASE, "workgroup");
          __builtin_amdgcn_wave_barrier();
          if (lane == 0) *const_cast<volatile unsigned *>(&X.pose_done[pair]) = c_front + 1;
        }
        SHC_TICK(25);
        if (prev_real) {
          resident_take_inputs<RPW, ROBOT_NONE, true>(A, c_back, prev_h0, prev_h1, wave, lane, tile, tile_i, dirty, held, st.n_robots);
          if (held.src_force != in_src_force || held.src_effort != in_src_effort) {
            in_at = leg_inputs_in_force<L, NJ>(A, st.legd, held.src_force, held.src_effort, ns, slot, wave * RPW + grp, leg);
            in_src_force = held.src_force, in_src_effort = held.src_effort;
          }
          LegInRing<NJ> in = in_at;
          if (FT::tipf(P)) in.prefetch_effort();
          SHC_TICK(31);
          const double *mb = &X.mailbox[pair][c_back & 1][0][lane];
          out.poser_tip = V3{mb[0], mb[64], mb[128]};
          if constexpr (!ODOM_WALKER) if (FT::odom(P)) {
            const V3 ov{mb[192], mb[256], mb[320]};
            if (__any(mb[384] != 0.0)) {
              if (mb[384] != 0.0) {
                if constexpr (ODOM_REGS) odometry_advance(odom[0], odom[1], odom[2], odom[3], P, ov.x, ov.y, ov.z, &odom_cache);
                else odometry_step(rb, P, ov.x, ov.y, ov.z, &odom_cache);
              }
            }
          }
          out.adm_delta = V3{0, 0, 0};
          if (FT::adm(P)) cycle_admittance<NJ>(s, out, P, in);
          s.word = 0;
          SHC_TICK(26);
          cycle_back<L, NJ, F>(s, out, C, leg, st.legd, ns, slot, nullptr, in, fb);
          SHC_TICK(27);
          asm volatile("s_waitcnt vmcnt(0)" ::: "memory");
          if (lane == 0) st_agent(A.progress + wave, u64(c_back));
          SHC_TICK(13);
          {
            typedef unsigned v4u __attribute__((ext_vector_type(4)));
            double flat[2 * NJ];
#pragma unroll
            for (int i = 0; i < NJ; ++i) flat[FD::Q + i] = s.q[i], flat[FD::QD + i] = s.qd[i];
            const unsigned soff = oslot * out_slot_bytes;
#ifdef SHC_ABLATE
            if (!(P.debug_skip & 4096))
#endif
            if (live) {
#pragma unroll
              for (int p = 0; p < NJ; ++p) {
                const u64 a = u64(__double_as_longlong(flat[2 * p])), b = u64(__double_as_longlong(flat[2 * p + 1]));
                const v4u w = {unsigned(a), unsigned(a >> 32), unsigned(b), unsigned(b >> 32)};
                __builtin_amdgcn_raw_buffer_store_b128(w, out_rsrc, unsigned((int64_t(p) * ns + slot) * 16), soff, 16 );
              }
            }
          }
          ++c_back;
          oslot = oslot + 1 == unsigned(A.depth) ? 0 : oslot + 1;
          SHC_TICK(28);
        }
        if (kind != IT_REAL) {
          asm volatile("s_waitcnt vmcnt(0)" ::: "memory");
          if (lane == 0) st_agent(A.progress + wave, u64(c_back));
        }
      }
      if (leader && kind != IT_EXIT && lane == 0) {
        X.ctrl[(k + 1) & 3][0] = u64(nk);
        X.ctrl[(k + 1) & 3][1] = nh0v;
        X.ctrl[(k + 1) & 3][2] = nh1v;
      }
      SHC_TICK(14);
      if (kind == IT_EXIT) break;
      SHC_R2_ITER_END(128, 19, 29, 24, 30, 25, 31, 26, 9, 10, 11, 12, 27, 13, 28, 14);
      if (kind == IT_REAL) ++c_front;
      prev_real = kind == IT_REAL;
      prev_h0 = h0, prev_h1 = h1;
      __syncthreads();
      ++k;
    }
  }
#undef SHC_R2_ITER_BEGIN
#undef SHC_R2_ITER_END
#undef SHC_R2_PHASES
#ifdef SHC_RES2_TIMING
  if (blockIdx.x == 1 && lane == 0 && pair == 0) {
    unsigned long long *dbg = reinterpret_cast<unsigned long long *>(A.ctl) + 8 + (walker ? 0 : 4);
    dbg[0] = tm_busy, dbg[1] = tm_real, dbg[2] = __builtin_readcyclecounter() - tm_total0, dbg[3] = k;
#ifndef SHC_RES2_BUSY_ONLY
    if (walker) {
      for (int i = 0; i < 32; ++i) dbg[8 + i] = (unsigned long long)shc_acc_lds[i];
    } else {
      for (int i = 0; i < 32; ++i) dbg[36 + i] = (unsigned long long)shc_acc_lds[32 + i];
    }
#endif
  }
#endif
  if (active && ODOM_REGS && FT::odom(P) && walker == ODOM_WALKER) {
#pragma unroll
    for (int i = 0; i < 4; ++i) rb.put(R::ODOM + i, odom[i]);
  }
  if (active) {
    if (walker) {
      X.stiff[pair][lane] = s.stiff;
    } else {
      X.ikfail[pair][lane] = s.word & LW_IKFAIL;
      if (POSE_SPLIT) {
        unsigned d = 0;
#pragma unroll
        for (unsigned b = 1; b <= DIRTY_LAST; b <<= 1)
          if (__any((dirty & b) != 0)) d |= b;
        if (lane == 0) X.model_dirty[pair] = d, X.model_seen[pair] = held.seen;
      }
      if (lane == 0) X.model_fault[pair] = held.fault ? 1u : 0u;
    }
  }
  __syncthreads();
  if (!active) return;
  if (walker) {
    if (POSE_SPLIT) dirty |= X.model_dirty[pair], held.seen |= X.model_seen[pair];
    if (X.model_fault[pair]) held.fault = true;
    if (c_front > 0) s.word = (s.word & ~LW_IKFAIL) | X.ikfail[pair][lane];
    {
      unsigned d = 0;
#pragma unroll
      for (unsigned b = 1; b <= DIRTY_LAST; b <<= 1)
        if (__any((dirty & b) != 0)) d |= b;
      dirty = d;
    }
    if (live) store_leg<NJ, F, ROLE_FRONT>(s, out, pk, st, P, slot, dirty);
    __builtin_amdgcn_wave_barrier();
    store_rob_fields<RPW, 0, R::PLANE>(tile, gtile, lane);
    if (dirty & DIRTY_WALK_PLANE) store_rob_fields<RPW, R::PLANE, R::VIN>(tile, gtile, lane);
    if (FT::manual(P) && manual_live && (dirty & DIRTY_MANUAL)) store_rob_fields<RPW, R::MPOSE, R::MANUAL_END>(tile, gtile, lane);
    if (FT::imu(P)) store_rob_fields<RPW, R::ABSE, R::GYRO>(tile, gtile, lane);
    if (FT::incl(P) && FT::autop(P)) store_rob_fields<RPW, R::APREV, R::APREV_END>(tile, gtile, lane);
    store_rob_fields<RPW, R::CPOSE, R::CPOSE_END>(tile, gtile, lane);
    if (FT::odom(P)) store_rob_fields<RPW, R::ODOM, R::ODOM_END>(tile, gtile, lane);
    if (lane < (R::I_POSE_PHASE + 1) * RPW) gtile_i[lane] = tile_i[lane];
    store_rob_fields<RPW, R::VIN, R::CORE_END>(tile, gtile, lane);
    if (held.seen & (1u << RG_IMU)) {
      store_rob_fields<RPW, R::GYRO, R::IMU_END>(tile, gtile, lane);
      store_rob_fields<RPW, R::IMUQ, R::IMUQ_END>(tile, gtile, lane);
    }
    if ((held.seen & (1u << RG_RESET)) && lane < RPW) gtile_i[R::I_RESET_MODE * RPW + lane] = tile_i[R::I_RESET_MODE * RPW + lane];
    if (lane == 0) {
      if (held.fault) __hip_atomic_fetch_or(&A.ctl->fault, 1ull, __ATOMIC_RELAXED, __HIP_MEMORY_SCOPE_AGENT);
      __hip_atomic_fetch_add(&A.ctl->exited, 1ull, __ATOMIC_RELAXED, __HIP_MEMORY_SCOPE_AGENT);
    }
  } else {
    s.stiff = X.stiff[pair][lane];
    if (live) {
      store_leg<NJ, F, ROLE_BACK>(s, out, pk, st, P, slot, 0);
      carry_leg_inputs<L, NJ>(A, st, held, ns, slot, leg);
    }
  }
}

}
```

### syropod_highlevel_controller_amd/csrc/shc_cycle_launch.hpp

```cpp
#pragma once

#include "shc_cycle.hpp"

#include <hip/hip_runtime.h>

namespace shc {

enum : int { RG_VEL = 0, RG_IMU = 1, RG_POSE = 2, RG_RESET = 3, RG_FORCE = 4, RG_EFFORT = 5, RG_COUNT = 6 };
enum : int { RIN_VEL = 0, RIN_IMU = 3, RIN_POSE = 10, RIN_COUNT = 16 };

constexpr int kResidentHeaders = 1024;
constexpr int kBoundSets = 4;
enum : int { BND_LIN = 0, BND_ANG = 1, BND_IMUQ = 2, BND_IMUW = 3, BND_FORCE = 4, BND_EFFORT = 5, BND_COUNT = 6 };
constexpr unsigned kResidentDirect = 1u << 15;
struct ResidentCtl {
  unsigned long long gate;
  unsigned long long exited;
  unsigned long long fault;
  unsigned long long pad[5];
  unsigned long long dbg[80];
};
struct ResidentHost {
  unsigned long long doorbell;
  unsigned long long stop;
  unsigned long long done;
  unsigned long long exited;
  unsigned long long heartbeat;
  unsigned long long fault;
  unsigned long long late_reads;
  unsigned long long pad_[1];
  unsigned long long records[kResidentHeaders * 2];
};
struct ResidentHeader {
  unsigned long long tag;
  unsigned short mask;
  unsigned char pos[RG_COUNT];
};
static_assert(sizeof(ResidentHeader) == 16, "header is read as two 8-byte words");
enum : unsigned long long { RESIDENT_EXIT_STOP = 1, RESIDENT_EXIT_IDLE = 2, RESIDENT_EXIT_MAX = 3, RESIDENT_EXIT_FAULT = 4 };

struct ResidentArgs {
  ResidentCtl *ctl;
  ResidentHost *host;
  unsigned long long *progress;
  ResidentHeader *headers;
  const double *bound[kBoundSets][BND_COUNT];
  const double *rin;
  const int32_t *rini;
  const double *force;
  const double *effort;
  double *out;
  int depth;
  unsigned max_cycles;
  unsigned long long idle_ticks;
  unsigned long long ticks_per_ms;
  int64_t n_waves;
  double touchdown_threshold, liftoff_threshold;
  unsigned batch_cycles, batch_mask;
  int64_t kstride[BND_COUNT];
  int64_t batch_wave0;
};

struct ResidentFit;
struct CycleLaunch {
  DevState st;
  const void *consts;
  const CycleParams *cp;
  unsigned rt_flags;
  bool generic;
  hipStream_t stream;
  unsigned grid;
  int block;
  int n_cycles;
  const ResidentArgs *resident;
  struct ResidentFit *fit;
  int64_t wave0;
  int half_steps;
};
struct ResidentFit {
  int supported;
  int blocks_per_cu;
  int two_wave;
  int batch;
};

#define SHC_FOR_EACH_MORPHOLOGY(X) X(3, 3) X(4, 3) X(4, 4) X(4, 5) X(5, 3) X(6, 3) X(6, 4) X(6, 5) X(7, 3) X(8, 3) X(8, 4) X(8, 5)
#define SHC_DECLARE_LAUNCHER(L_, NJ_) bool shc_launch_cycle_##L_##_##NJ_(const CycleLaunch &a);
SHC_FOR_EACH_MORPHOLOGY(SHC_DECLARE_LAUNCHER)
#undef SHC_DECLARE_LAUNCHER

}
```

### syropod_highlevel_controller_amd/csrc/shc_cycle_select.hpp

```cpp
#pragma once

#include "shc_cycle.hpp"

#include <utility>

#ifndef SHC_GENERIC_LOOP_FORMS
#define SHC_GENERIC_LOOP_FORMS 0
#endif

namespace shc {

constexpr unsigned F_C2 = F_MANUAL | F_ODOM;
constexpr unsigned F_C3 = F_MANUAL | F_IMU | F_ADM | F_ODOM;
constexpr bool is_baseline_morphology(int L, int NJ) { return (L == 6 && NJ == 3) || (L == 8 && NJ == 5); }

static inline unsigned select_features(int L, int NJ, const CycleParams &c, unsigned rt_flags, bool generic) {
  const bool baseline = is_baseline_morphology(L, NJ), exact = !generic;
  const unsigned f = (c.manual_posing ? F_MANUAL : 0) | (c.auto_posing ? F_AUTO : 0) | (c.inclination_posing ? F_INCL : 0) |
                     (c.imu_posing ? F_IMU : 0) | (c.admittance_control ? F_ADM : 0) | (c.tip_force ? F_TIPF : 0) | (c.odometry ? F_ODOM : 0);
  const bool rough = c.rough_terrain != 0, talign = c.tip_align != 0, mlegs = (rt_flags & RT_MANUAL_LEGS) != 0;
  const bool terrain = rough || talign || mlegs;
  if (NJ > 3 && (c.gravity_aligned || (mlegs && c.joint_control == 2))) {
    if (exact && !terrain) {
      if (f == F_C2) return F_C2 | F_ROT;
      if (baseline && (f == (F_C2 | F_TIPF) || f == F_C3)) return f | F_ROT;
    }
    return terrain ? F_DYN | F_ROT | F_TERRAIN : F_DYN | F_ROT;
  }
  if (NJ == 3 && mlegs && c.joint_control == 2) return rough || talign ? F_DYN | F_ROT | F_TERRAIN : F_DYN | F_ROT | F_MLEGS;
  if (terrain) {
    const bool only_rough = rough && !talign && !mlegs, only_mlegs = mlegs && !rough && !talign;
    const bool only_talign = NJ <= 3 && talign && !rough && !mlegs;
    if (baseline && exact && (f & ~F_TIPF) == F_C2) {
      if (only_rough) return f | F_ROUGH;
      if (only_talign) return f | F_TALIGN;
    }
    return only_rough ? F_DYN | F_ROUGH : only_mlegs ? F_DYN | F_MLEGS : only_talign ? F_DYN | F_TALIGN : F_DYN | F_TERRAIN;
  }
  if (exact) {
    if (f == F_C2) return F_C2;
    if (baseline && (f == (F_C2 | F_TIPF) || f == F_C3 || f == (F_C3 | F_TIPF))) return f;
  }
  return F_DYN;
}

template <unsigned... Fs>
using FeatureList = std::integer_sequence<unsigned, Fs...>;
template <int L, int NJ>
constexpr auto kernel_table() {
  if constexpr (L == 6 && NJ == 3)
    return FeatureList<F_DYN, F_C3, F_C3 | F_TIPF, F_C2, F_C2 | F_TIPF, F_DYN | F_TERRAIN, F_DYN | F_TALIGN, F_DYN | F_MLEGS, F_DYN | F_ROUGH,
                       F_C2 | F_TALIGN, F_C2 | F_TIPF | F_TALIGN, F_C2 | F_ROUGH, F_C2 | F_TIPF | F_ROUGH, F_DYN | F_ROT | F_MLEGS,
                       F_DYN | F_ROT | F_TERRAIN>{};
  else if constexpr (L == 8 && NJ == 5)
    return FeatureList<F_DYN, F_C3, F_C3 | F_TIPF, F_C2, F_C2 | F_TIPF, F_DYN | F_TERRAIN, F_DYN | F_MLEGS, F_DYN | F_ROUGH, F_C2 | F_ROUGH,
                       F_C2 | F_TIPF | F_ROUGH, F_DYN | F_ROT, F_DYN | F_ROT | F_TERRAIN, F_C3 | F_ROT, F_C2 | F_TIPF | F_ROT, F_C2 | F_ROT>{};
  else if constexpr (NJ == 3)
    return FeatureList<F_DYN, F_C2, F_DYN | F_TERRAIN, F_DYN | F_TALIGN, F_DYN | F_MLEGS, F_DYN | F_ROUGH, F_DYN | F_ROT | F_MLEGS,
                       F_DYN | F_ROT | F_TERRAIN>{};
  else
    return FeatureList<F_DYN, F_C2, F_DYN | F_TERRAIN, F_DYN | F_MLEGS, F_DYN | F_ROUGH, F_DYN | F_ROT, F_DYN | F_ROT | F_TERRAIN, F_C2 | F_ROT>{};
}
template <int L, int NJ>
using KernelTable = decltype(kernel_table<L, NJ>());

constexpr bool has_resident(unsigned F) { return (F & F_MLEGS) == 0 && (SHC_GENERIC_LOOP_FORMS || (F & F_DYN) == 0 || (F & (F_TERRAIN | F_ROT)) == 0); }
constexpr bool has_batch(unsigned F) { return (F & F_MLEGS) == 0 && (SHC_GENERIC_LOOP_FORMS || (F & F_DYN) == 0); }
constexpr bool has_two_wave(unsigned F) { return has_resident(F) && (F & (F_TERRAIN | F_ROT)) == 0; }
constexpr bool has_half_kernels(unsigned F) { return (F & F_ROT) != 0 && (F & (F_DYN | F_TERRAIN | F_MLEGS | F_AUTO)) == 0; }

}
```

### syropod_highlevel_controller_amd/csrc/shc_resident.hpp

```cpp

struct Resident {
  bool active = false;
  int depth = 0;
  ResidentArgs args{};
  ResidentHost *host = nullptr;
  ResidentHost *host_dev = nullptr;
  ResidentCtl *ctl = nullptr;
  unsigned long long *progress = nullptr;
  ResidentHeader *headers = nullptr;
  double *rin = nullptr, *force = nullptr, *effort = nullptr, *out = nullptr, *stage = nullptr;
  int32_t *rini = nullptr;
  size_t stage_bytes = 0;
  static constexpr int kPinSlots = 4;
  unsigned *post_blocks_done = nullptr;
  char *pin = nullptr, *pin_dev = nullptr;
  hipEvent_t pin_ev[kPinSlots] = {};
  unsigned long long pin_uses = 0;
  hipStream_t in_stream = nullptr;
  hipStream_t loop_stream = nullptr;
  hipEvent_t loop_ev = nullptr;
  unsigned long long published = 0;
  unsigned long long posted = 0;
  unsigned long long posts[RG_COUNT] = {};
  std::vector<unsigned long long> post_cycle[RG_COUNT];
  unsigned max_cycles = 0;
  unsigned long long wall_khz = 100000;
  bool poisoned = false;
  bool stream_doorbell_pending = false;
  unsigned groups_posted = 0;
  bool two_wave = false;
  long long direct_last = -1;
};

__global__ void resident_doorbell_kernel(ResidentHost *host, unsigned long long value) {
  __hip_atomic_store(&host->doorbell, value, __ATOMIC_RELAXED, __HIP_MEMORY_SCOPE_SYSTEM);
}

struct ResidentPost {
  const double *lin, *ang, *imu_q, *imu_w, *tvi, *rvi, *force, *effort;
  const int32_t *reset;
  int pos[RG_COUNT];
  unsigned mask;
  unsigned long long cycle;
  unsigned long long doorbell;
  ResidentHost *host;
  unsigned *blocks_done;
};
__global__ void resident_post_kernel(ResidentPost pp, ResidentArgs A, ResidentHeader *headers, double *rin, int32_t *rini, double *force, double *effort,
                                     int64_t n, int L, int NJ, int64_t n_slots) {
  const int64_t t = int64_t(blockIdx.x) * blockDim.x + threadIdx.x;
  const int rpw = 64 / L;
  auto put = [](double *p, double v) {
    __hip_atomic_store(reinterpret_cast<unsigned long long *>(p), (unsigned long long)__double_as_longlong(v), __ATOMIC_RELAXED, __HIP_MEMORY_SCOPE_AGENT);
  };
  if (t < n) {
    const int64_t w = t / rpw;
    const int r = int(t - w * rpw);
    auto rec = [&](int grp, int field) { return rin + ((int64_t(pp.pos[grp]) * A.n_waves + w) * RIN_COUNT + field) * rpw + r; };
    if (pp.mask & (1u << RG_VEL)) {
      put(rec(RG_VEL, RIN_VEL), pp.lin[t * 2]);
      put(rec(RG_VEL, RIN_VEL + 1), pp.lin[t * 2 + 1]);
      put(rec(RG_VEL, RIN_VEL + 2), pp.ang[t]);
    }
    if (pp.mask & (1u << RG_IMU)) {
      const Quat qn = normalized(Quat{pp.imu_q[t * 4], pp.imu_q[t * 4 + 1], pp.imu_q[t * 4 + 2], pp.imu_q[t * 4 + 3]});
      put(rec(RG_IMU, RIN_IMU + 0), qn.w);
      put(rec(RG_IMU, RIN_IMU + 1), qn.x);
      put(rec(RG_IMU, RIN_IMU + 2), qn.y);
      put(rec(RG_IMU, RIN_IMU + 3), qn.z);
      for (int k = 0; k < 3; ++k) put(rec(RG_IMU, RIN_IMU + 4 + k), pp.imu_w[t * 3 + k]);
    }
    if (pp.mask & (1u << RG_POSE)) {
      for (int k = 0; k < 3; ++k) put(rec(RG_POSE, RIN_POSE + k), pp.tvi[t * 3 + k]);
      for (int k = 0; k < 3; ++k) put(rec(RG_POSE, RIN_POSE + 3 + k), pp.rvi[t * 3 + k]);
    }
    if (pp.mask & (1u << RG_RESET))
      __hip_atomic_store(reinterpret_cast<unsigned long long *>(rini) + ((int64_t(pp.pos[RG_RESET]) * A.n_waves + w) * rpw + r),
                         (unsigned long long)(unsigned)pp.reset[t], __ATOMIC_RELAXED, __HIP_MEMORY_SCOPE_AGENT);
  }
  if (t < n * L && (pp.mask & ((1u << RG_FORCE) | (1u << RG_EFFORT)))) {
    const int64_t rob = t / L;
    const int leg = int(t - rob * L);
    const int64_t slot = slot_of(rob, leg, L);
    if (pp.mask & (1u << RG_FORCE)) {
      double *base = force + int64_t(pp.pos[RG_FORCE]) * 2 * n_slots * 2;
      for (int k = 0; k < 3; ++k) put(base + leg_field_index(k, slot, n_slots), pp.force[t * 3 + k]);
    }
    if (pp.mask & (1u << RG_EFFORT)) {
      const int nje = (NJ + 1) & ~1;
      double *base = effort + int64_t(pp.pos[RG_EFFORT]) * (nje / 2) * n_slots * 2;
      for (int k = 0; k < NJ; ++k) put(base + leg_field_index(k, slot, n_slots), pp.effort[t * NJ + k]);
    }
  }
  if (t == 0) {
    unsigned long long h1 = pp.mask & 0xffffu;
    for (int gi = 0; gi < RG_COUNT; ++gi) h1 |= (unsigned long long)(pp.pos[gi] & 0xff) << (16 + 8 * gi);
    unsigned long long *hp = reinterpret_cast<unsigned long long *>(headers + (pp.cycle & (kResidentHeaders - 1)));
    __hip_atomic_store(hp + 1, h1, __ATOMIC_RELAXED, __HIP_MEMORY_SCOPE_AGENT);
    __hip_atomic_store(hp, pp.cycle + 1, __ATOMIC_RELAXED, __HIP_MEMORY_SCOPE_AGENT);
  }
  if (pp.doorbell != 0) {
    __threadfence();
    __syncthreads();
    if (threadIdx.x == 0) {
      const unsigned arrived = __hip_atomic_fetch_add(pp.blocks_done, 1u, __ATOMIC_ACQ_REL, __HIP_MEMORY_SCOPE_AGENT);
      if (arrived == gridDim.x - 1) {
        __hip_atomic_store(pp.blocks_done, 0u, __ATOMIC_RELAXED, __HIP_MEMORY_SCOPE_AGENT);
        __threadfence_system();
        __hip_atomic_store(&pp.host->doorbell, pp.doorbell, __ATOMIC_RELEASE, __HIP_MEMORY_SCOPE_SYSTEM);
      }
    }
  }
}

static void resident_free(Resident *r) {
  if (!r) return;
  if (r->host) (void)hipHostFree(r->host);
  (void)hipFree(r->ctl);
  (void)hipFree(r->progress);
  (void)hipFree(r->headers);
  (void)hipFree(r->rin);
  (void)hipFree(r->rini);
  (void)hipFree(r->force);
  (void)hipFree(r->effort);
  (void)hipFree(r->out);
  (void)hipFree(r->stage);
  (void)hipFree(r->post_blocks_done);
  if (r->pin) (void)hipHostFree(r->pin);
  for (hipEvent_t ev : r->pin_ev)
    if (ev) (void)hipEventDestroy(ev);
  if (r->in_stream) (void)hipStreamDestroy(r->in_stream);
  if (r->loop_stream) (void)hipStreamDestroy(r->loop_stream);
  if (r->loop_ev) (void)hipEventDestroy(r->loop_ev);
  delete r;
}

static inline unsigned long long host_load(const unsigned long long *p) { return __atomic_load_n(p, __ATOMIC_ACQUIRE); }
static inline void host_store(unsigned long long *p, unsigned long long v) { __atomic_store_n(p, v, __ATOMIC_RELEASE); }
static double now_seconds() {
  timespec ts;
  clock_gettime(CLOCK_MONOTONIC, &ts);
  return double(ts.tv_sec) + 1e-9 * double(ts.tv_nsec);
}
template <typename Pred>
static bool spin_until(Pred pred, double timeout_s) {
  const double t0 = now_seconds();
  for (unsigned it = 0;; ++it) {
    if (pred()) return true;
    const double dt = now_seconds() - t0;
    if (dt > timeout_s) return false;
    if (dt > 200e-6 && (it & 63) == 0) sched_yield();
  }
}

static int resident_require(shc_engine *e, bool active) {
  if (!e) return fail(SHC_ERR_INVALID_ARG, "engine is NULL");
  if (active && !(e->res && e->res->active)) return fail(SHC_ERR_INVALID_ARG, "the engine is not in resident mode (shc_engine_resident_begin)");
  return SHC_OK;
}

extern "C" int shc_engine_resident_bind_inputs(shc_engine *e, int set, const shc_cycle_inputs *arrays) {
  if (!e) return fail(SHC_ERR_INVALID_ARG, "engine is NULL");
  if (e->res && e->res->active) return fail(SHC_ERR_BUSY, "resident mode: input sets are bound while the loop is not running");
  if (set < 0 || set >= kBoundSets) return fail(SHC_ERR_INVALID_ARG, "input set 0 .. 3");
  if (arrays && (arrays->linear_xy == nullptr) != (arrays->angular == nullptr)) return fail(SHC_ERR_INVALID_ARG, "linear_xy and angular are bound together");
  if (arrays && (arrays->imu_orientation_wxyz == nullptr) != (arrays->imu_angular_velocity == nullptr)) return fail(SHC_ERR_INVALID_ARG, "the two IMU arrays are bound together");
  if (arrays && (arrays->pose_translation_velocity || arrays->pose_rotation_velocity || arrays->pose_reset_mode))
    return fail(SHC_ERR_INVALID_ARG, "input sets carry velocity, IMU, tip force and joint effort");
  const double *row[BND_COUNT] = {nullptr, nullptr, nullptr, nullptr, nullptr, nullptr};
  if (arrays) {
    row[BND_LIN] = arrays->linear_xy, row[BND_ANG] = arrays->angular, row[BND_IMUQ] = arrays->imu_orientation_wxyz, row[BND_IMUW] = arrays->imu_angular_velocity;
    row[BND_FORCE] = arrays->tip_force, row[BND_EFFORT] = arrays->joint_effort;
  }
  memcpy(e->bound_inputs[set], row, sizeof row);
  return SHC_OK;
}

static int resident_fit(const shc_engine *e, ResidentFit &fit) {
  fit = ResidentFit{0, 0, 0, 0};
  CycleLaunch a = cycle_launch(e);
  a.fit = &fit;
  return launch_cycle_for(e, a);
}

extern "C" int shc_engine_resident_begin(shc_engine *e, int ring_depth, int64_t max_cycles, int idle_timeout_ms) {
  if (!e) return fail(SHC_ERR_INVALID_ARG, "engine is NULL");
  if (e->res && e->res->active) return fail(SHC_ERR_BUSY, "resident mode is already active");
  if (ring_depth < 2 || ring_depth > 255) return fail(SHC_ERR_INVALID_ARG, "ring_depth must be 2..255");
  if (max_cycles < 1 || max_cycles > 0x7ffffffe) return fail(SHC_ERR_INVALID_ARG, "max_cycles must be 1..2^31-2");
  if (idle_timeout_ms < 0 || idle_timeout_ms > 600000) return fail(SHC_ERR_INVALID_ARG, "idle_timeout_ms must be 0..600000");
  if (e->starting_up) return fail(SHC_ERR_UNSUPPORTED, "resident mode starts from a running engine (finish the start-up first)");
  if (adjust_needs_stepped_cycle(e))
    return fail(SHC_ERR_UNSUPPORTED, "resident mode cannot start while an adjusted parameter waits for its cycle (the posing part of the next cycle runs on "
                                     "the old value): call shc_engine_step(e, 1) once first");
  {
    const int rc_remap = adjust_serve_now(e);
    if (rc_remap != SHC_OK) return rc_remap;
  }
  HIP_TRY(hipSetDevice(e->device));
  {
    const int rc = join_side(e);
    if (rc != SHC_OK) return rc;
  }
  ResidentFit fit;
  {
    const int rc = resident_fit(e, fit);
    if (rc != SHC_OK) return rc;
  }
  if (!fit.supported)
    return fail(SHC_ERR_UNSUPPORTED, (e->rt_flags & RT_MANUAL_LEGS)
                                         ? "resident mode: this configuration runs on a manual-leg kernel (a leg has been toggled / planner mode), which has no resident form"
                                         : "resident mode: this configuration runs on a runtime-flag kernel with rough terrain / tip-align / tip-rotation logic, whose resident "
                                           "form is not part of this build (SHC_GENERIC_LOOP_FORMS=1 builds it); use shc_engine_step or shc_engine_step_k");
  hipDeviceProp_t prop;
  HIP_TRY(hipGetDeviceProperties(&prop, e->device));
  constexpr int kXcds = 8;
  const int64_t capacity = int64_t(fit.blocks_per_cu) * (prop.multiProcessorCount - kXcds);
  if (e->n_waves + 1 > capacity)
    return fail(SHC_ERR_UNSUPPORTED, "resident mode: the batch needs " + std::to_string(e->n_waves + 1) + " co-resident wavefronts, this device holds " +
                                         std::to_string(capacity) + " of this kernel (" + std::to_string(fit.blocks_per_cu) + " per compute unit); use shc_engine_step");
  const int NJE = (e->NJ + 1) & ~1;
  const size_t out_slot_bytes = size_t(e->NJ) * e->n_slots * 16;
  if (out_slot_bytes * size_t(ring_depth) >= (size_t(1) << 31)) return fail(SHC_ERR_INVALID_ARG, "ring_depth x batch: the output ring must stay below 2 GiB");
  HIP_TRY(hipStreamSynchronize(e->stream));
  if (e->res && e->res->depth != ring_depth) {
    resident_free(e->res);
    e->res = nullptr;
  }
  if (!e->res) {
    Resident *r = new Resident();
    e->res = r;
    r->depth = ring_depth;
    const int rpw = 64 / e->L;
    auto bail = [&](hipError_t err, const char *what) {
      resident_free(r);
      e->res = nullptr;
      return fail(SHC_ERR_HIP, std::string(what) + ": " + hipGetErrorString(err));
    };
    hipError_t err;
    if ((err = hipHostMalloc(reinterpret_cast<void **>(&r->host), sizeof(ResidentHost), hipHostMallocMapped | hipHostMallocCoherent)) != hipSuccess)
      return bail(err, "hipHostMalloc(ResidentHost)");
    if ((err = hipHostGetDevicePointer(reinterpret_cast<void **>(&r->host_dev), r->host, 0)) != hipSuccess) return bail(err, "hipHostGetDevicePointer");
    if ((err = hipStreamCreateWithFlags(&r->in_stream, hipStreamNonBlocking)) != hipSuccess) return bail(err, "hipStreamCreate");
    {
      int least = 0, greatest = 0;
      if (hipDeviceGetStreamPriorityRange(&least, &greatest) != hipSuccess) least = 0;
      if ((err = hipStreamCreateWithPriority(&r->loop_stream, hipStreamNonBlocking, least)) != hipSuccess) return bail(err, "hipStreamCreate");
    }
    if ((err = hipEventCreateWithFlags(&r->loop_ev, hipEventDisableTiming)) != hipSuccess) return bail(err, "hipEventCreate");
    r->stage_bytes = size_t(e->n) * (16 * 8 + 8) + size_t(e->n) * e->L * (3 + e->NJ) * 8 + 256;
    const size_t D = size_t(ring_depth);
    if ((err = hipMalloc(&r->ctl, sizeof(ResidentCtl))) != hipSuccess) return bail(err, "hipMalloc");
    if ((err = hipMalloc(&r->progress, size_t(e->n_waves) * 8)) != hipSuccess) return bail(err, "hipMalloc");
    if ((err = hipMalloc(&r->headers, sizeof(ResidentHeader) * kResidentHeaders)) != hipSuccess) return bail(err, "hipMalloc");
    if ((err = hipMalloc(&r->rin, D * e->n_waves * RIN_COUNT * rpw * 8)) != hipSuccess) return bail(err, "hipMalloc");
    if ((err = hipMalloc(&r->rini, D * e->n_waves * rpw * 8)) != hipSuccess) return bail(err, "hipMalloc");
    if ((err = hipMalloc(&r->force, D * 2 * e->n_slots * 16)) != hipSuccess) return bail(err, "hipMalloc");
    if ((err = hipMalloc(&r->effort, D * (NJE / 2) * e->n_slots * 16)) != hipSuccess) return bail(err, "hipMalloc");
    if ((err = hipMalloc(&r->out, D * out_slot_bytes)) != hipSuccess) return bail(err, "hipMalloc");
    if ((err = hipMalloc(&r->stage, r->stage_bytes)) != hipSuccess) return bail(err, "hipMalloc");
    if ((err = hipMalloc(&r->post_blocks_done, 64)) != hipSuccess) return bail(err, "hipMalloc");
    if ((err = hipMemsetAsync(r->post_blocks_done, 0, 64, e->stream)) != hipSuccess) return bail(err, "hipMemset");
    if ((err = hipHostMalloc(reinterpret_cast<void **>(&r->pin), r->stage_bytes * Resident::kPinSlots, hipHostMallocMapped)) != hipSuccess)
      return bail(err, "hipHostMalloc(input staging)");
    if ((err = hipHostGetDevicePointer(reinterpret_cast<void **>(&r->pin_dev), r->pin, 0)) != hipSuccess) return bail(err, "hipHostGetDevicePointer");
    for (hipEvent_t &ev : r->pin_ev)
      if ((err = hipEventCreateWithFlags(&ev, hipEventDisableTiming)) != hipSuccess) return bail(err, "hipEventCreate");
    for (int gi = 0; gi < RG_COUNT; ++gi) r->post_cycle[gi].assign(D, 0);
  }
  Resident *r = e->res;
  {
    ResidentCtl ctl0{};
    ctl0.gate = (unsigned long long)(unsigned(max_cycles)) << 32;
    HIP_TRY(hipMemcpyAsync(r->ctl, &ctl0, sizeof ctl0, hipMemcpyHostToDevice, e->stream));
    HIP_TRY(hipStreamSynchronize(e->stream));
  }
  HIP_TRY(hipMemsetAsync(r->progress, 0, size_t(e->n_waves) * 8, e->stream));
  HIP_TRY(hipMemsetAsync(r->headers, 0, sizeof(ResidentHeader) * kResidentHeaders, e->stream));
  memset(r->host, 0, sizeof(ResidentHost));
  r->host->stop = ~0ull;
  __sync_synchronize();
  r->published = r->posted = 0;
  r->direct_last = -1;
  r->groups_posted = 0;
  r->stream_doorbell_pending = false;
  for (int gi = 0; gi < RG_COUNT; ++gi) {
    r->posts[gi] = 0;
    std::fill(r->post_cycle[gi].begin(), r->post_cycle[gi].end(), 0ull);
  }
  r->max_cycles = unsigned(max_cycles);
  ResidentArgs &A = r->args;
  A.ctl = r->ctl;
  A.host = r->host_dev;
  A.progress = r->progress;
  A.headers = r->headers;
  memcpy(A.bound, e->bound_inputs, sizeof A.bound);
  A.rin = r->rin;
  A.rini = r->rini;
  A.force = r->force;
  A.effort = r->effort;
  A.out = r->out;
  A.depth = ring_depth;
  A.max_cycles = r->max_cycles;
  int wall_khz = 0;
  if (hipDeviceGetAttribute(&wall_khz, hipDeviceAttributeWallClockRate, e->device) != hipSuccess || wall_khz <= 0) wall_khz = 100000;
  r->wall_khz = (unsigned long long)wall_khz;
  A.idle_ticks = (unsigned long long)(idle_timeout_ms ? idle_timeout_ms : 5000) * r->wall_khz;
  A.ticks_per_ms = r->wall_khz;
  A.n_waves = e->n_waves;
  A.touchdown_threshold = e->params.touchdown_threshold;
  A.liftoff_threshold = e->params.liftoff_threshold;
  e->plan_poser_tips_current = false;
  const bool two_wave = fit.two_wave && !(e->features & SHC_FEAT_RESIDENT_ONE_WAVE) && (e->n_waves + 1) / 2 + 1 <= prop.multiProcessorCount;
  r->two_wave = two_wave;
  HIP_TRY(hipEventRecord(r->loop_ev, e->stream));
  HIP_TRY(hipStreamWaitEvent(r->loop_stream, r->loop_ev, 0));
  CycleLaunch a = cycle_launch(e);
  a.stream = r->loop_stream, a.resident = &A;
  a.grid = two_wave ? unsigned((e->n_waves + 1) / 2 + 1) : unsigned(e->n_waves + 1), a.block = two_wave ? 256 : 64;
  {
    const int rc = launch_cycle_for(e, a);
    if (rc != SHC_OK) return rc;
  }
  HIP_TRY(hipGetLastError());
  r->active = true;
  return SHC_OK;
}

static int resident_wait_direct_installed(Resident *r) {
  if (r->direct_last < 0) return SHC_OK;
  const unsigned long long need = (unsigned long long)r->direct_last + 1;
  if (!spin_until([&] { return host_load(&r->host->done) >= need || host_load(&r->host->exited) != 0; }, 5.0))
    return fail(SHC_ERR_TIMEOUT, "resident mode: a direct post is still waiting to run");
  r->direct_last = -1;
  return SHC_OK;
}

static int resident_alive(Resident *r) {
  if (const unsigned long long why = host_load(&r->host->exited))
    return fail(SHC_ERR_TIMEOUT, std::string("resident mode: the device loop has stopped by itself (") +
                                     (why == RESIDENT_EXIT_IDLE ? "idle timeout" : why == RESIDENT_EXIT_MAX ? "max_cycles" : why == RESIDENT_EXIT_FAULT ? "fault" : "stop") +
                                     " after " + std::to_string(host_load(&r->host->done)) + " cycles): call shc_engine_resident_end");
  return SHC_OK;
}

extern "C" int shc_engine_resident_post(shc_engine *e, const shc_cycle_inputs *in, int64_t *cycle) {
  int rc = resident_require(e, true);
  if (rc != SHC_OK) return rc;
  Resident *r = e->res;
  if ((rc = resident_alive(r)) != SHC_OK) return rc;
  if (!in) return fail(SHC_ERR_INVALID_ARG, "inputs is NULL");
  if ((in->linear_xy == nullptr) != (in->angular == nullptr)) return fail(SHC_ERR_INVALID_ARG, "linear_xy and angular are posted together");
  if ((in->imu_orientation_wxyz == nullptr) != (in->imu_angular_velocity == nullptr)) return fail(SHC_ERR_INVALID_ARG, "the two IMU arrays are posted together");
  if ((in->pose_translation_velocity == nullptr) != (in->pose_rotation_velocity == nullptr))
    return fail(SHC_ERR_INVALID_ARG, "the two pose input arrays are posted together");
  unsigned mask = 0;
  if (in->linear_xy) mask |= 1u << RG_VEL;
  if (in->imu_orientation_wxyz) mask |= 1u << RG_IMU;
  if (in->pose_translation_velocity) mask |= 1u << RG_POSE;
  if (in->pose_reset_mode) mask |= 1u << RG_RESET;
  if (in->tip_force) mask |= 1u << RG_FORCE;
  if (in->joint_effort) mask |= 1u << RG_EFFORT;
  if ((mask & ((1u << RG_POSE) | (1u << RG_RESET))) && !(e->rt_flags & RT_MANUAL_LIVE))
    return fail(SHC_ERR_UNSUPPORTED, "pose inputs: give the engine one (shc_engine_set_pose_input / set_pose_reset_mode) before shc_engine_resident_begin");
  if ((mask & (1u << RG_EFFORT)) && !(e->rt_flags & RT_EFFORT_LIVE))
    return fail(SHC_ERR_UNSUPPORTED, "joint efforts: give the engine one (shc_engine_set_joint_effort) before shc_engine_resident_begin");
  const unsigned long long c = r->posted;
  if (c < r->published) return fail(SHC_ERR_INVALID_ARG, "resident mode: this cycle has already been published without inputs");
  if (c >= r->max_cycles) return fail(SHC_ERR_INVALID_ARG, "resident mode: past max_cycles");
  HIP_TRY(hipSetDevice(e->device));
  const double patience = 5.0;
  if (c >= kResidentHeaders && !spin_until([&] { return host_load(&r->host->done) > c - kResidentHeaders; }, patience))
    return fail(SHC_ERR_TIMEOUT, "resident mode: 1024 posted cycles are waiting to run");
  if (in->direct) {
    const int set = in->direct - 1;
    if (set < 0 || set >= kBoundSets) return fail(SHC_ERR_INVALID_ARG, "direct: bound input set 1 .. 4");
    if (mask & ((1u << RG_POSE) | (1u << RG_RESET))) return fail(SHC_ERR_INVALID_ARG, "direct posts carry velocity, IMU, tip force and joint effort; post pose inputs / reset modes the ordinary way");
    if (mask == 0) return fail(SHC_ERR_INVALID_ARG, "direct post without inputs (use shc_engine_resident_publish)");
    const int need[RG_COUNT] = {BND_LIN, BND_IMUQ, -1, -1, BND_FORCE, BND_EFFORT};
    for (int gi = 0; gi < RG_COUNT; ++gi)
      if ((mask & (1u << gi)) && (need[gi] < 0 || !r->args.bound[set][need[gi]]))
        return fail(SHC_ERR_INVALID_ARG, "direct post: that group is not part of the bound input set (shc_engine_resident_bind_inputs before shc_engine_resident_begin)");
    if (r->published < c) {
      const int rc2 = shc_engine_resident_publish(e, int64_t(c - r->published));
      if (rc2 != SHC_OK) return rc2;
    }
    const unsigned long long tag = c + 1;
    volatile unsigned long long *rec = r->host->records + size_t(c & (kResidentHeaders - 1)) * 2;
    rec[1] = (unsigned long long)mask | ((unsigned long long)set << 16) | ((tag & 0xffffull) << 48);
    host_store(const_cast<unsigned long long *>(&rec[0]), tag);
    r->groups_posted |= mask;
    r->posted = r->published = c + 1;
    r->direct_last = (long long)c;
    if (cycle) *cycle = int64_t(c);
    return SHC_OK;
  }
  ResidentPost pp{};
  pp.mask = mask;
  pp.cycle = c;
  for (int gi = 0; gi < RG_COUNT; ++gi) {
    if (!(mask & (1u << gi))) continue;
    const unsigned long long k = r->posts[gi];
    pp.pos[gi] = int(k % r->depth);
    if (k >= (unsigned long long)r->depth) {
      const unsigned long long successor_cycle = r->post_cycle[gi][(k + 1) % r->depth];
      if (!spin_until([&] { return host_load(&r->host->done) >= successor_cycle || host_load(&r->host->exited) != 0; }, patience))
        return fail(SHC_ERR_TIMEOUT, "resident mode: ring_depth posted input sets are waiting to be consumed (publish them)");
    }
  }
  size_t off = 0;
  const int pin_slot = int(r->pin_uses % Resident::kPinSlots);
  if (!in->on_device && r->pin_uses >= (unsigned long long)Resident::kPinSlots) HIP_TRY(hipEventSynchronize(r->pin_ev[pin_slot]));
  auto dev = [&](const void *src, size_t bytes, const void **out) -> int {
    if (in->on_device) {
      *out = src;
      return SHC_OK;
    }
    if (off + bytes > r->stage_bytes) return fail(SHC_ERR_INVALID_ARG, "staging buffer too small");
    const size_t at = size_t(pin_slot) * r->stage_bytes + off;
    memcpy(r->pin + at, src, bytes);
    *out = r->pin_dev + at;
    off += (bytes + 15) & ~size_t(15);
    return SHC_OK;
  };
  const size_t n = size_t(e->n), nl = n * e->L;
#define STAGE(field, member, bytes)                                                              \
  if (in->member) {                                                                              \
    const void *d_;                                                                              \
    if ((rc = dev(in->member, bytes, &d_)) != SHC_OK) return rc;                                 \
    pp.field = reinterpret_cast<decltype(pp.field)>(d_);                                         \
  }
  STAGE(lin, linear_xy, n * 16)
  STAGE(ang, angular, n * 8)
  STAGE(imu_q, imu_orientation_wxyz, n * 32)
  STAGE(imu_w, imu_angular_velocity, n * 24)
  STAGE(tvi, pose_translation_velocity, n * 24)
  STAGE(rvi, pose_rotation_velocity, n * 24)
  STAGE(reset, pose_reset_mode, n * 4)
  STAGE(force, tip_force, nl * 24)
  STAGE(effort, joint_effort, nl * e->NJ * 8)
#undef STAGE
  const int64_t threads = (mask & ((1u << RG_FORCE) | (1u << RG_EFFORT))) ? int64_t(nl) : int64_t(n);
  const bool publish = in->publish != 0;
  if (publish) {
    if ((rc = resident_wait_direct_installed(r)) != SHC_OK) return rc;
    pp.doorbell = c + 1;
    pp.host = r->host_dev;
    pp.blocks_done = r->post_blocks_done;
  }
  resident_post_kernel<<<dim3((unsigned)((threads + 63) / 64)), dim3(64), 0, r->in_stream>>>(pp, r->args, r->headers, r->rin, r->rini, r->force, r->effort,
                                                                                              e->n, e->L, e->NJ, e->n_slots);
  HIP_TRY(hipGetLastError());
  if (!in->on_device) {
    HIP_TRY(hipEventRecord(r->pin_ev[pin_slot], r->in_stream));
    r->pin_uses++;
  }
  for (int gi = 0; gi < RG_COUNT; ++gi)
    if (mask & (1u << gi)) {
      r->post_cycle[gi][r->posts[gi] % r->depth] = c;
      r->posts[gi]++;
    }
  r->groups_posted |= mask;
  r->posted = c + 1;
  if (publish) r->published = c + 1;
  r->stream_doorbell_pending = true;
  if (cycle) *cycle = int64_t(c);
  return SHC_OK;
}

extern "C" int shc_engine_resident_publish(shc_engine *e, int64_t n_cycles) {
  int rc = resident_require(e, true);
  if (rc != SHC_OK) return rc;
  Resident *r = e->res;
  if ((rc = resident_alive(r)) != SHC_OK) return rc;
  if (n_cycles < 0) return fail(SHC_ERR_INVALID_ARG, "n_cycles < 0");
  if (n_cycles == 0) return SHC_OK;
  if (r->published + (unsigned long long)n_cycles > r->max_cycles) return fail(SHC_ERR_INVALID_ARG, "resident mode: past max_cycles");
  if ((rc = resident_wait_direct_installed(r)) != SHC_OK) return rc;
  r->published += (unsigned long long)n_cycles;
  if (r->posted < r->published) r->posted = r->published;
  if (r->stream_doorbell_pending) {
    HIP_TRY(hipSetDevice(e->device));
    if (hipStreamQuery(r->in_stream) == hipSuccess) {
      r->stream_doorbell_pending = false;
    } else {
      resident_doorbell_kernel<<<dim3(1), dim3(1), 0, r->in_stream>>>(r->host_dev, r->published);
      HIP_TRY(hipGetLastError());
      return SHC_OK;
    }
  }
  host_store(&r->host->doorbell, r->published);
  return SHC_OK;
}

extern "C" int shc_engine_resident_wait(shc_engine *e, int64_t cycles, int timeout_ms) {
  int rc = resident_require(e, true);
  if (rc != SHC_OK) return rc;
  Resident *r = e->res;
  if (cycles < 0 || (unsigned long long)cycles > r->published) return fail(SHC_ERR_INVALID_ARG, "resident mode: waiting for cycles that were not published");
  const unsigned long long want = (unsigned long long)cycles;
  if (!spin_until([&] { return host_load(&r->host->done) >= want || host_load(&r->host->exited) != 0; }, timeout_ms > 0 ? timeout_ms * 1e-3 : 10.0))
    return fail(SHC_ERR_TIMEOUT, "resident mode: the published cycles did not complete in time");
  if (host_load(&r->host->done) < want) return fail(SHC_ERR_TIMEOUT, "resident mode: the device loop stopped before these cycles ran");
  return SHC_OK;
}

extern "C" int shc_engine_resident_get_joint_state(shc_engine *e, int64_t cycle, double *q, double *qd, int on_device) {
  int rc = resident_require(e, true);
  if (rc != SHC_OK) return rc;
  Resident *r = e->res;
  const unsigned long long done = host_load(&r->host->done);
  if (cycle < 0 || (unsigned long long)cycle >= done) return fail(SHC_ERR_INVALID_ARG, "resident mode: that cycle has not completed (shc_engine_resident_wait)");
  if (r->published > (unsigned long long)cycle + r->depth)
    return fail(SHC_ERR_INVALID_ARG, "resident mode: that cycle's outputs may have been overwritten (ring_depth newer cycles were published)");
  HIP_TRY(hipSetDevice(e->device));
  const double *slot = r->out + size_t(cycle % r->depth) * size_t(e->NJ) * e->n_slots * 2;
  const int64_t threads = e->n * e->L;
  for (int which = 0; which < 2; ++which) {
    double *dst = which ? qd : q;
    if (!dst) continue;
    double *d = on_device ? dst : r->stage;
    gather_leg_kernel<<<dim3((unsigned)((threads + 63) / 64)), dim3(64), 0, r->in_stream>>>(d, slot, e->n_slots, e->n, e->L, e->NJ,
                                                                                            which ? LEG_FIELD(e, QD) : LEG_FIELD(e, Q));
    HIP_TRY(hipGetLastError());
    if (!on_device) {
      HIP_TRY(hipMemcpyAsync(dst, d, size_t(threads) * e->NJ * 8, hipMemcpyDeviceToHost, r->in_stream));
      HIP_TRY(hipStreamSynchronize(r->in_stream));
    }
  }
  if (on_device) HIP_TRY(hipStreamSynchronize(r->in_stream));
  return SHC_OK;
}

__global__ void resident_wait_done_kernel(const ResidentCtl *ctl, ResidentHost *host, unsigned long long want, unsigned long long timeout_ticks) {
  const unsigned long long t0 = wall_clock64();
  auto done = [&] { return __hip_atomic_load(&ctl->pad[1], __ATOMIC_ACQUIRE, __HIP_MEMORY_SCOPE_AGENT); };
  for (;;) {
    if (done() >= want) return;
    if (__hip_atomic_load(&ctl->pad[2], __ATOMIC_ACQUIRE, __HIP_MEMORY_SCOPE_AGENT) != 0 && done() < want) break;
    if (wall_clock64() - t0 > timeout_ticks) break;
    __builtin_amdgcn_s_sleep(8);
  }
  __hip_atomic_fetch_add(&host->late_reads, 1ull, __ATOMIC_RELAXED, __HIP_MEMORY_SCOPE_SYSTEM);
}

extern "C" int shc_engine_resident_get_joint_state_async(shc_engine *e, int64_t cycle, double *q, double *qd, int timeout_ms) {
  int rc = resident_require(e, true);
  if (rc != SHC_OK) return rc;
  Resident *r = e->res;
  if ((rc = resident_alive(r)) != SHC_OK) return rc;
  if (cycle < 0 || (unsigned long long)cycle >= r->max_cycles) return fail(SHC_ERR_INVALID_ARG, "resident mode: no such cycle (max_cycles)");
  if (r->published > (unsigned long long)cycle + r->depth)
    return fail(SHC_ERR_INVALID_ARG, "resident mode: that cycle's outputs may have been overwritten (ring_depth newer cycles were published)");
  HIP_TRY(hipSetDevice(e->device));
  const unsigned long long ticks = (unsigned long long)(timeout_ms > 0 ? timeout_ms : 5000) * r->wall_khz;
  resident_wait_done_kernel<<<dim3(1), dim3(1), 0, e->stream>>>(r->ctl, r->host_dev, (unsigned long long)cycle + 1, ticks);
  HIP_TRY(hipGetLastError());
  const double *slot = r->out + size_t(cycle % r->depth) * size_t(e->NJ) * e->n_slots * 2;
  const int64_t threads = e->n * e->L;
  for (int which = 0; which < 2; ++which) {
    double *dst = which ? qd : q;
    if (!dst) continue;
    gather_leg_kernel<<<dim3((unsigned)((threads + 63) / 64)), dim3(64), 0, e->stream>>>(dst, slot, e->n_slots, e->n, e->L, e->NJ,
                                                                                         which ? LEG_FIELD(e, QD) : LEG_FIELD(e, Q));
    HIP_TRY(hipGetLastError());
  }
  return SHC_OK;
}

extern "C" int shc_engine_resident_status(shc_engine *e, int64_t *published, int64_t *completed, int32_t *running) {
  int rc = resident_require(e, false);
  if (rc != SHC_OK) return rc;
  Resident *r = e->res;
  const bool active = r && r->active;
  if (published) *published = active ? int64_t(r->published) : 0;
  if (completed) *completed = active ? int64_t(host_load(&r->host->done)) : 0;
  if (running) *running = active && host_load(&r->host->exited) == 0 ? 1 : 0;
  return SHC_OK;
}

extern "C" int shc_engine_resident_end(shc_engine *e, int64_t *cycles_run) {
  int rc = resident_require(e, true);
  if (rc != SHC_OK) return rc;
  Resident *r = e->res;
  HIP_TRY(hipSetDevice(e->device));
  HIP_TRY(hipStreamSynchronize(r->in_stream));
  const int direct_rc = resident_wait_direct_installed(r);
  const std::string direct_msg = direct_rc != SHC_OK ? std::string(shc_last_error()) : std::string();
  if (direct_rc == SHC_OK) host_store(&r->host->doorbell, r->published);
  host_store(&r->host->stop, direct_rc == SHC_OK ? r->published : 0ull);
  const bool answered = spin_until([&] { return host_load(&r->host->exited) != 0; }, r->poisoned ? 5.0 : 30.0);
  if (!answered) {
    r->poisoned = true;
    return fail(SHC_ERR_TIMEOUT, "resident mode: the device loop did not answer the stop request in time; the engine stays in resident mode - call "
                                 "shc_engine_resident_end again");
  }
  hipError_t err = hipStreamSynchronize(r->loop_stream);
  if (err == hipSuccess) err = hipStreamSynchronize(e->stream);
  r->active = false;
  r->poisoned = false;
#ifdef SHC_RES2_TIMING
  if (err == hipSuccess) {
    ResidentCtl c;
    (void)hipMemcpy(&c, r->ctl, sizeof c, hipMemcpyDeviceToHost);
    for (int w = 0; w < 2; ++w)
      fprintf(stderr, "[res2 timing] %s: %.0f clocks busy per steady REAL iteration (%llu of them), loop %llu clocks, %llu iterations\n", w ? "model " : "walker",
              c.dbg[4 * w + 1] ? double(c.dbg[4 * w]) / double(c.dbg[4 * w + 1]) : 0.0, c.dbg[4 * w + 1], c.dbg[4 * w + 2], c.dbg[4 * w + 3]);
#ifndef SHC_RES2_BUSY_ONLY
    const int order[] = {20, 21, 2, 3, 4, 5, 6, 7, 16, 8, 17, 15, 29, 22, 23};
    const char *wname[] = {"control words (LDS) read", "inputs of the cycle taken", "cycle_front entry", "robot word / command read, stop predicates", "(pose elsewhere)", "getLimit",
                           "velocity shaping", "walk state machine", "stepper (stride, Bezier, tip)", "tip rotation / iteratePhase / planes / leg word", "wait for the pose flag",
                           "pose read + updateStance", "control input for the next pose published", "mailbox written", "to the barrier"};
    const double its = c.dbg[1] ? double(c.dbg[1]) : 1.0;
    fprintf(stderr, "[res2 timing] walker of pair 0, mean clocks per phase:\n");
    for (int i = 0; i < int(sizeof(order) / sizeof(int)); ++i) fprintf(stderr, "[res2 timing]   walker t%-2d %-58s %7.0f\n", order[i], wname[i], double(c.dbg[8 + order[i]]) / its);
    const int morder[] = {29, 24, 30, 25, 31, 26, 9, 10, 11, 12, 27, 13, 28, 14};
    const char *mname[] = {"control words (LDS) read", "leader: gate, what the next iteration is, header prefetch issued", "pose inputs of the cycle taken",
                           "updateCurrentPose of the walker's cycle + flag", "leg inputs in force, joint efforts prefetched", "mailbox read, odometry, admittance",
                           "cycle_back entry (desired tip)", "IK step + joint update", "sin / cos, chain, Jacobian", "model tip, tip force", "cycle_back exit",
                           "wait for the previous stores + progress word", "output-ring stores issued", "control words written (leader: waits for its loads)"};
    const double mits = c.dbg[5] ? double(c.dbg[5]) : 1.0;
    fprintf(stderr, "[res2 timing] model wavefront of pair 0 (the leader), mean clocks per phase:\n");
    for (int i = 0; i < int(sizeof(morder) / sizeof(int)); ++i) fprintf(stderr, "[res2 timing]   model  t%-2d %-58s %7.0f\n", morder[i], mname[i], double(c.dbg[40 + morder[i]]) / mits);
#endif
  }
#endif
  const unsigned long long reason = host_load(&r->host->exited), done = host_load(&r->host->done);
  if (cycles_run) *cycles_run = int64_t(done);
  if (r->groups_posted & (1u << RG_FORCE)) e->rt_flags |= RT_TOUCHDOWN;
  if (err != hipSuccess) return fail(SHC_ERR_HIP, std::string("hipStreamSynchronize: ") + hipGetErrorString(err));
  if (direct_rc != SHC_OK) return fail(direct_rc, direct_msg + " (the loop was stopped after " + std::to_string(done) + " cycles)");
  if (reason == RESIDENT_EXIT_FAULT || host_load(&r->host->fault) != 0)
    return fail(SHC_ERR_HIP, "resident mode: a wavefront gave up waiting for the relay; restore the engine from a snapshot");
  if (host_load(&r->host->late_reads) != 0)
    return fail(SHC_ERR_TIMEOUT, "resident mode: a stream-ordered read (shc_engine_resident_get_joint_state_async) gave up waiting for its cycle");
  if (!((reason == RESIDENT_EXIT_STOP || reason == RESIDENT_EXIT_MAX) && done == r->published))
    return fail(SHC_ERR_TIMEOUT, std::string("resident mode: the device loop had stopped by itself (") +
                                     (reason == RESIDENT_EXIT_IDLE ? "idle timeout" : reason == RESIDENT_EXIT_MAX ? "max_cycles" : "unknown") + ") after " +
                                     std::to_string(done) + " of " + std::to_string(r->published) + " published cycles");
  return SHC_OK;
}

static int step_k_out_ring(shc_engine *e, int K) {
  const size_t need = size_t(K) * size_t(e->NJ) * size_t(e->n_slots) * 16;
  if (e->k_out && e->k_out_bytes >= need) return SHC_OK;
  if (e->k_out) {
    const int rc = join_side(e);
    if (rc != SHC_OK) return rc;
    HIP_TRY(hipStreamSynchronize(e->stream));
    (void)hipFree(e->k_out);
    e->k_out = nullptr, e->k_out_bytes = 0;
  }
  HIP_TRY(hipMalloc(reinterpret_cast<void **>(&e->k_out), need));
  e->k_out_bytes = need;
  return SHC_OK;
}

__global__ void copy_joint_planes_kernel(double2 *dst, const double2 *src, int64_t count);
static int step_k_serial(shc_engine *e, int K, const shc_cycle_inputs *in) {
  const int64_t n = e->n, slot = int64_t(e->NJ) * e->n_slots;
  for (int k = 0; k < K; ++k) {
    int rc = SHC_OK;
    if (in && in->linear_xy) rc = shc_engine_set_velocity(e, in->linear_xy + k * n * 2, in->angular + k * n, 1);
    if (rc == SHC_OK && in && in->imu_orientation_wxyz) rc = shc_engine_set_imu(e, in->imu_orientation_wxyz + k * n * 4, in->imu_angular_velocity + k * n * 3, 1);
    if (rc == SHC_OK && in && in->tip_force) rc = shc_engine_set_tip_force(e, in->tip_force + k * n * e->L * 3, 1);
    if (rc == SHC_OK && in && in->joint_effort) rc = shc_engine_set_joint_effort(e, in->joint_effort + k * n * e->L * e->NJ, 1);
    if (rc == SHC_OK) rc = shc_engine_step(e, 1);
    if (rc == SHC_OK) rc = join_side(e);
    if (rc != SHC_OK) return rc;
    copy_joint_planes_kernel<<<dim3((unsigned)((slot + 255) / 256)), dim3(256), 0, e->stream>>>(reinterpret_cast<double2 *>(e->k_out) + k * slot,
                                                                                              reinterpret_cast<const double2 *>(e->st.legd), slot);
    HIP_TRY(hipGetLastError());
  }
  e->k_out_cycles = K;
  return SHC_OK;
}

extern "C" int shc_engine_step_k(shc_engine *e, int n_cycles, const shc_cycle_inputs *in) {
  SHC_ENTER(e);
  if (n_cycles < 1 || n_cycles > 4096) return fail(SHC_ERR_INVALID_ARG, "shc_engine_step_k: 1 .. 4096 cycles per launch");
  if (e->starting_up) return fail(SHC_ERR_UNSUPPORTED, "shc_engine_step_k starts from a running engine (finish the start-up first)");
  unsigned mask = 0;
  if (in) {
    if (!in->on_device) return fail(SHC_ERR_INVALID_ARG, "shc_engine_step_k: the K-deep input arrays are device arrays (on_device = 1)");
    if ((in->linear_xy == nullptr) != (in->angular == nullptr)) return fail(SHC_ERR_INVALID_ARG, "linear_xy and angular are given together");
    if ((in->imu_orientation_wxyz == nullptr) != (in->imu_angular_velocity == nullptr)) return fail(SHC_ERR_INVALID_ARG, "the two IMU arrays are given together");
    if (in->pose_translation_velocity || in->pose_rotation_velocity || in->pose_reset_mode)
      return fail(SHC_ERR_UNSUPPORTED, "shc_engine_step_k carries velocity, IMU, tip force and joint effort; give pose inputs / reset modes with their setters before the call (held for the K cycles)");
    if (in->linear_xy) mask |= 1u << RG_VEL;
    if (in->imu_orientation_wxyz) mask |= 1u << RG_IMU;
    if (in->tip_force) mask |= 1u << RG_FORCE;
    if (in->joint_effort) mask |= 1u << RG_EFFORT;
  }
  HIP_TRY(hipSetDevice(e->device));
  const bool split = e->n_waves >= kSplitWaves && !(e->features & SHC_FEAT_SINGLE_STREAM);
  if (!split || ((mask & (1u << RG_EFFORT)) && !(e->rt_flags & RT_EFFORT_LIVE))) {
    const int rc = join_side(e);
    if (rc != SHC_OK) return rc;
  }
  if (mask & (1u << RG_EFFORT)) {
    const int rc = effort_live(e);
    if (rc != SHC_OK) return rc;
  }
  ResidentFit fit;
  {
    const int rc = resident_fit(e, fit);
    if (rc != SHC_OK) return rc;
  }
  if (size_t(e->NJ) * e->n_slots * 16 * size_t(n_cycles) >= (size_t(1) << 31))
    return fail(SHC_ERR_INVALID_ARG, "shc_engine_step_k: cycles x batch - the output ring must stay below 2 GiB (fewer cycles per launch)");
  {
    const int rc = step_k_out_ring(e, n_cycles);
    if (rc != SHC_OK) return rc;
  }
  if (!fit.batch || (e->features & SHC_FEAT_STEP_K_SERIAL)) return step_k_serial(e, n_cycles, in);
  int k0 = 0;
  if (adjust_pending(e)) {
    const int rc = step_k_serial(e, 1, in);
    if (rc != SHC_OK) return rc;
    if (n_cycles == 1) return SHC_OK;
    k0 = 1;
  }
  e->plan_poser_tips_current = false;
  ResidentArgs A{};
  A.kstride[BND_LIN] = e->n * 2, A.kstride[BND_ANG] = e->n, A.kstride[BND_IMUQ] = e->n * 4, A.kstride[BND_IMUW] = e->n * 3;
  A.kstride[BND_FORCE] = e->n * e->L * 3, A.kstride[BND_EFFORT] = e->n * e->L * e->NJ;
  if (in) {
    const auto row = [&](const double *a, int which) { return a ? a + k0 * A.kstride[which] : a; };
    A.bound[0][BND_LIN] = row(in->linear_xy, BND_LIN), A.bound[0][BND_ANG] = row(in->angular, BND_ANG);
    A.bound[0][BND_IMUQ] = row(in->imu_orientation_wxyz, BND_IMUQ), A.bound[0][BND_IMUW] = row(in->imu_angular_velocity, BND_IMUW);
    A.bound[0][BND_FORCE] = row(in->tip_force, BND_FORCE), A.bound[0][BND_EFFORT] = row(in->joint_effort, BND_EFFORT);
  }
  A.out = e->k_out + size_t(k0) * size_t(e->NJ) * e->n_slots * 2;
  A.depth = n_cycles - k0;
  A.max_cycles = unsigned(n_cycles - k0);
  A.batch_cycles = unsigned(n_cycles - k0);
  A.batch_mask = mask;
  A.n_waves = e->n_waves;
  A.idle_ticks = 0, A.ticks_per_ms = 100000;
  A.touchdown_threshold = e->params.touchdown_threshold;
  A.liftoff_threshold = e->params.liftoff_threshold;
  const LaunchGeometry g = launch_geometry(e);
  CycleLaunch a = cycle_launch(e);
  a.block = g.block, a.resident = &A;
  int rc;
  if (!split) {
    a.grid = g.grid(e->n_waves);
    if ((rc = launch_cycle_for(e, a)) != SHC_OK) return rc;
    HIP_TRY(hipGetLastError());
  } else {
    if ((rc = ensure_split_streams(e)) != SHC_OK) return rc;
    HIP_TRY(hipEventRecord(e->ev_main, e->stream));
    for (int h = 0; h < 2; ++h) {
      HIP_TRY(hipStreamWaitEvent(e->half_stream[h], e->ev_main, 0));
      A.batch_wave0 = h ? g.half : 0;
      a.stream = e->half_stream[h];
      a.grid = g.grid(h ? e->n_waves - g.half : g.half);
      if ((rc = launch_cycle_for(e, a)) != SHC_OK) return rc;
      HIP_TRY(hipGetLastError());
    }
    e->main_dirty = false;
    e->side_busy = true;
  }
  e->k_out_cycles = n_cycles;
  if (mask & (1u << RG_FORCE)) e->rt_flags |= RT_TOUCHDOWN;
  return SHC_OK;
}

extern "C" int shc_engine_get_step_k_joint_state(shc_engine *e, int k, double *q, double *qd, int on_device) {
  SHC_ENTER_JOINED(e);
  if (!e->k_out || k < 0 || k >= e->k_out_cycles) return fail(SHC_ERR_INVALID_ARG, "shc_engine_get_step_k_joint_state: cycle 0 .. K - 1 of the latest shc_engine_step_k");
  HIP_TRY(hipSetDevice(e->device));
  const double *slot = e->k_out + size_t(k) * size_t(e->NJ) * e->n_slots * 2;
  const int64_t threads = e->n * e->L;
  for (int which = 0; which < 2; ++which) {
    double *dst = which ? qd : q;
    if (!dst) continue;
    double *d = on_device ? dst : e->d_stage;
    if (!on_device && size_t(threads) * e->NJ * 8 > e->stage_bytes) return fail(SHC_ERR_INVALID_ARG, "staging buffer too small");
    gather_leg_kernel<<<dim3((unsigned)((threads + 63) / 64)), dim3(64), 0, e->stream>>>(d, slot, e->n_slots, e->n, e->L, e->NJ, which ? LEG_FIELD(e, QD) : LEG_FIELD(e, Q));
    HIP_TRY(hipGetLastError());
    if (!on_device) {
      HIP_TRY(hipMemcpyAsync(dst, d, size_t(threads) * e->NJ * 8, hipMemcpyDeviceToHost, e->stream));
      HIP_TRY(hipStreamSynchronize(e->stream));
    }
  }
  return SHC_OK;
}
```

Before: 1.578 billion.

## Add a third helper wavefront that takes pose, odometry and leader gating off the model wave

Adds a 384-thread, three-role form of the two-wavefront resident kernel for 6-leg 3-joint robots with specific feature sets. A helper wavefront per pair now runs the pose update, odometry and leader gate/header prefetch, and reduces the walk-plane control candidate from raw leg words. This leaves the model wavefront with only IK and joint work, shortening the critical path of the pipeline. The cost is an extra wave per block (more registers and LDS, fewer blocks per CU) and more LDS traffic between roles. It is on by default where it applies and can be disabled with an environment variable.

Result: faster. 1.644 billion (median of 6 runs) (+4.2%).

```diff
diff --git a/syropod_highlevel_controller_amd/csrc/shc_cycle.hpp b/syropod_highlevel_controller_amd/csrc/shc_cycle.hpp
--- a/syropod_highlevel_controller_amd/csrc/shc_cycle.hpp
+++ b/syropod_highlevel_controller_amd/csrc/shc_cycle.hpp
@@ -174,9 +174,9 @@
 }
 #define SHC_PHASE_FENCE() do { if constexpr (phase_fences<L, NJ, F>()) __builtin_amdgcn_sched_barrier(0); } while (0)
 #if defined(SHC_RES2_TIMING) && !defined(SHC_RES2_BUSY_ONLY)
-__shared__ long long shc_ticks_lds[64];
-__shared__ long long shc_acc_lds[64];
-#define SHC_TICK(i) do { __builtin_amdgcn_sched_barrier(0); if (blockIdx.x == 1 && (threadIdx.x == 0 || threadIdx.x == 128)) shc_ticks_lds[(threadIdx.x >> 7) * 32 + (i)] = __builtin_readcyclecounter(); __builtin_amdgcn_sched_barrier(0); } while (0)
+__shared__ long long shc_ticks_lds[96];
+__shared__ long long shc_acc_lds[96];
+#define SHC_TICK(i) do { __builtin_amdgcn_sched_barrier(0); if (blockIdx.x == 1 && (threadIdx.x & 127) == 0) shc_ticks_lds[(threadIdx.x >> 7) * 32 + (i)] = __builtin_readcyclecounter(); __builtin_amdgcn_sched_barrier(0); } while (0)
 #else
 #define SHC_TICK(i) do {} while (0)
 #endif
diff --git a/syropod_highlevel_controller_amd/csrc/shc_cycle_inst.hip b/syropod_highlevel_controller_amd/csrc/shc_cycle_inst.hip
--- a/syropod_highlevel_controller_amd/csrc/shc_cycle_inst.hip
+++ b/syropod_highlevel_controller_amd/csrc/shc_cycle_inst.hip
@@ -35,6 +35,7 @@
     a.fit->supported = has_resident(F) ? 1 : 0;
     a.fit->batch = has_batch(F) ? 1 : 0;
     a.fit->two_wave = has_two_wave(F) ? 1 : 0;
+    a.fit->helper_wave = has_helper_wave(L, NJ, F) ? 1 : 0;
     a.fit->blocks_per_cu = 0;
     if constexpr (has_resident(F)) {
       int blocks = 0;
@@ -45,6 +46,13 @@
     if constexpr (has_batch(F)) {
       note_kernel("batch", L, NJ, F);
       shc_batch_kernel<L, NJ, F><<<dim3(a.grid), dim3(a.block), wave_bytes * (a.block / 64), a.stream>>>(a.st, (const SharedConsts<L, NJ> *)a.consts, *a.resident, a.rt_flags);
+    }
+  } else if (a.block == 384) {
+    if constexpr (has_helper_wave(L, NJ, F)) {
+      static_assert(has_two_wave(F), "the three-role form is a form of the two-wavefront pipeline");
+      note_kernel("resident3", L, NJ, F);
+      shc_resident2_kernel<L, NJ, F, true><<<dim3(a.grid), dim3(384), 2 * wave_bytes + sizeof(Resident3Lds<L, NJ>), a.stream>>>(
+          a.st, (const SharedConsts<L, NJ> *)a.consts, *a.resident, a.rt_flags);
     }
   } else if (a.block == 256) {
     if constexpr (has_two_wave(F)) {
diff --git a/syropod_highlevel_controller_amd/csrc/shc_cycle_kernel.hpp b/syropod_highlevel_controller_amd/csrc/shc_cycle_kernel.hpp
--- a/syropod_highlevel_controller_amd/csrc/shc_cycle_kernel.hpp
+++ b/syropod_highlevel_controller_amd/csrc/shc_cycle_kernel.hpp
@@ -4,6 +4,8 @@
 #include "shc_cycle_launch.hpp"
 
 #include <hip/hip_runtime.h>
+
+#include <type_traits>
 
 namespace shc {
 
@@ -948,13 +950,19 @@
   int ikfail[2][64];
   unsigned long long ctrl[4][4];
 };
-
-template <int L, int NJ, unsigned F>
-__global__ void __launch_bounds__(256, 1) shc_resident2_kernel(DevState st, const SharedConsts<L, NJ> *gc, ResidentArgs A, unsigned rt_flags) {
+template <int L, int NJ>
+struct Resident3Lds : Resident2Lds<L, NJ> {
+  int leg_word[2][2][64];
+  unsigned back_seen[2];
+};
+
+template <int L, int NJ, unsigned F, bool HELPER = false>
+__global__ void __launch_bounds__(HELPER ? 384 : 256, 1) shc_resident2_kernel(DevState st, const SharedConsts<L, NJ> *gc, ResidentArgs A, unsigned rt_flags) {
   using R = RobotFields;
   using FD = Fields<NJ>;
   using FT = Feat<F>;
   constexpr int RPW = 64 / L;
+  constexpr int kThreads = HELPER ? 384 : 256;
   if (blockIdx.x == 0) {
     if (threadIdx.x < 64) resident_relay<PART_GATE>(A);
     else if (threadIdx.x < 128) resident_relay<PART_DONE>(A);
@@ -963,12 +971,13 @@
   __shared__ SharedConsts<L, NJ> C;
   extern __shared__ double wave_lds[];
   constexpr int kWaveDoubles = R::COUNT * RPW + PK_COUNT * 64 + (R::I_COUNT * RPW + 1) / 2;
-  Resident2Lds<L, NJ> &X = *reinterpret_cast<Resident2Lds<L, NJ> *>(wave_lds + 2 * kWaveDoubles);
+  using Lds = std::conditional_t<HELPER, Resident3Lds<L, NJ>, Resident2Lds<L, NJ>>;
+  Lds &X = *reinterpret_cast<Lds *>(wave_lds + 2 * kWaveDoubles);
   const bool manual_live = (rt_flags & RT_MANUAL_LIVE) != 0;
   const int lane = threadIdx.x & 63;
   const int wib = __builtin_amdgcn_readfirstlane(threadIdx.x >> 6);
   const int pair = wib & 1;
-  const bool walker = wib < 2, leader = wib == 2;
+  const bool walker = HELPER ? (wib >> 1) == 1 : wib < 2, helper = HELPER && wib >= 4, leader = wib == (HELPER ? 4 : 2);
   const int64_t wave = (int64_t(blockIdx.x) - 1) * 2 + pair;
   const bool active = wave < A.n_waves;
   const int64_t rob0 = wave * RPW;
@@ -994,7 +1003,7 @@
     const int n16 = FT::autop(GP) ? n16_all : n16_core;
     const double2 *src = reinterpret_cast<const double2 *>(gc);
     double2 *dst = reinterpret_cast<double2 *>(&C);
-    for (int i = threadIdx.x; i < n16; i += 256) dst[i] = src[i];
+    for (int i = threadIdx.x; i < n16; i += kThreads) dst[i] = src[i];
   }
   LegLoad<NJ> ll;
   if (active) {
@@ -1003,7 +1012,7 @@
       for (int i = lane; i < R::COUNT * RPW; i += 64) tile[i] = gtile[i];
       for (int i = lane; i < R::I_COUNT * RPW; i += 64) tile_i[i] = gtile_i[i];
       load_leg_finish<NJ, ROLE_FRONT>(s, pk, ll);
-    } else {
+    } else if (!helper) {
       load_leg_issue<NJ, F, ROLE_BACK>(ll, st, GP, slot);
       load_leg_finish<NJ, ROLE_BACK>(s, pk, ll);
     }
@@ -1021,7 +1030,7 @@
   LegOut out;
   out.poser_tip = out.model_tip = out.adm_delta = V3{0, 0, 0};
   s.tipx = V3{1, 0, 0};
-  if (active && !walker) {
+  if (active && !walker && !helper) {
 #pragma unroll
     for (int k = 0; k < NJ; ++k) sincos_joint(C.leg[leg].link_th[k] + s.q[k], &s.sn[k], &s.cs[k]);
     if (FT::adm(P) || LegRegs<NJ>::kKeepJacobian) {
@@ -1047,7 +1056,8 @@
         mb[7 * 64] = pp.x, mb[8 * 64] = pp.y, mb[9 * 64] = pp.z, mb[10 * 64] = pn.x, mb[11 * 64] = pn.y, mb[12 * 64] = pn.z;
       }
     }
-    X.pose_c[pair][cycle & 1][lane] = walk_plane_control_candidate<L, NJ>(s.word, C, P, swing_c_count_u);
+    if constexpr (HELPER) X.leg_word[pair][cycle & 1][lane] = s.word;
+    else X.pose_c[pair][cycle & 1][lane] = walk_plane_control_candidate<L, NJ>(s.word, C, P, swing_c_count_u);
   };
   if (POSE_SPLIT && walker && active) publish_for_pose(0, true);
   const int64_t ns = st.n_slots;
@@ -1063,18 +1073,21 @@
   fb.uf = load_uni_flags(C.P);
   OdomCache odom_cache;
   Pose owpp_cache = pose_identity();
-  if (POSE_SPLIT && active && !walker) owpp_cache = rb.getpose(R::OWPP);
+  const bool poser = HELPER ? helper : !walker;
+  if (POSE_SPLIT && active && poser) owpp_cache = rb.getpose(R::OWPP);
   constexpr bool ODOM_REGS = NJ <= 3;
   constexpr bool ODOM_WALKER = NJ > 3 || (F & (F_ADM | F_IMU | F_INCL | F_AUTO | F_DYN)) != 0;
+  static_assert(!HELPER || (POSE_SPLIT && !ODOM_WALKER && ODOM_REGS), "the helper takes the pose and the odometry off the MODEL wavefront");
+  const bool odom_mine = ODOM_WALKER ? walker : poser;
   double odom[4] = {0.0, 0.0, 1.0, 0.0};
-  if (ODOM_REGS && FT::odom(P) && active && walker == ODOM_WALKER) {
+  if (ODOM_REGS && FT::odom(P) && active && odom_mine) {
 #pragma unroll
     for (int i = 0; i < 4; ++i) odom[i] = rb.get(R::ODOM + i);
   }
 #ifdef SHC_RES2_TIMING
   long long tm_busy = 0, tm_total0 = __builtin_readcyclecounter(), tm_real = 0;
 #ifndef SHC_RES2_BUSY_ONLY
-  if (threadIdx.x < 64) shc_acc_lds[threadIdx.x] = 0;
+  if (threadIdx.x < 96) shc_acc_lds[threadIdx.x] = 0;
 #endif
 #endif
 #ifdef SHC_RES2_TIMING
@@ -1098,6 +1111,82 @@
 #endif
   LegInRing<NJ> in_at;
   int in_src_force = -1000, in_src_effort = -1000;
+  const auto leader_decide = [&](const int kind, int &nk, u64 &nh0v, u64 &nh1v) __attribute__((always_inline)) {
+    u64 gate;
+    if (kind == IT_BUBBLE) {
+      __builtin_amdgcn_s_sleep(2);
+      gate = uni64(ld_agent(&A.ctl->gate));
+    } else {
+      gate = uni64(gate_pref);
+    }
+    const unsigned db = unsigned(gate), sp = unsigned(gate >> 32);
+    const unsigned cn = c_front + (kind == IT_REAL ? 1u : 0u);
+    nk = cn >= sp ? IT_EXIT : (cn < db ? IT_REAL : IT_BUBBLE);
+    if (nk == IT_BUBBLE) {
+      const u64 now = wall_clock64();
+      if (bubble_since == 0) bubble_since = now;
+      else if (now - bubble_since > emergency_ticks) nk = IT_EXIT, held.fault = true;
+    } else {
+      bubble_since = 0;
+    }
+    if (nk == IT_REAL) {
+      const u64 *hp = reinterpret_cast<const u64 *>(A.headers + (cn & (kResidentHeaders - 1)));
+      nh0v = ld_agent(hp);
+      nh1v = ld_agent(hp + 1);
+    }
+    if (kind == IT_BUBBLE) gate_pref = gate;
+    else gate_pref = ld_agent(&A.ctl->gate);
+  };
+  const auto leader_announce = [&](const int nk, const u64 nh0v, const u64 nh1v) __attribute__((always_inline)) {
+    X.ctrl[(k + 1) & 3][0] = u64(nk);
+    X.ctrl[(k + 1) & 3][1] = nh0v;
+    X.ctrl[(k + 1) & 3][2] = nh1v;
+  };
+  const auto pose_of_cycle = [&](const u64 h0, const u64 h1) __attribute__((always_inline)) {
+    if constexpr (!POSE_SPLIT) return;
+    else {
+    resident_take_inputs<RPW, ROBOT_POSE, false>(A, c_front, h0, h1, wave, lane, tile, tile_i, dirty, held, st.n_robots);
+    SHC_TICK(30);
+    double pose_c = -1.0;
+    if constexpr (HELPER) {
+      const double c_own = walk_plane_control_candidate<L, NJ>(X.leg_word[pair][c_front & 1][lane], C, P, swing_c_count_u);
+#pragma unroll
+      for (int j = 0; j < L; ++j) {
+        const double cj = g.get(c_own, j);
+        pose_c = cj >= 0.0 ? cj : pose_c;
+      }
+    } else {
+#pragma unroll
+      for (int j = 0; j < L; ++j) {
+        const double cj = X.pose_c[pair][c_front & 1][g.base + j];
+        pose_c = cj >= 0.0 ? cj : pose_c;
+      }
+    }
+    int lw[L] = {};
+    const double *mb = &X.mailbox[pair][c_front & 1][0][lane];
+    const V3 plane_prev{mb[7 * 64], mb[8 * 64], mb[9 * 64]}, pnorm_prev{mb[10 * 64], mb[11 * 64], mb[12 * 64]};
+    int rword_unused = 0;
+    Pose ap = pose_identity(), la = pose_identity();
+#ifdef SHC_ABLATE
+    if (!(P.debug_skip & 2048))
+#endif
+    (void)cycle_pose<L, NJ, F, true>(s, C, P, C.leg[leg], rb, g, leg, lw, rword_unused, 0, dirty, manual_live, ap, la, plane_prev, pnorm_prev, fb.uf.swing_c_count, 0,
+                                     &owpp_cache, &pose_c);
+    __builtin_amdgcn_fence(__ATOMIC_RELEASE, "workgroup");
+    __builtin_amdgcn_wave_barrier();
+    if (lane == 0) *const_cast<volatile unsigned *>(&X.pose_done[pair]) = c_front + 1;
+    }
+  };
+  const auto odometry_of_cycle = [&](const double *mb) __attribute__((always_inline)) {
+    const V3 ov{mb[192], mb[256], mb[320]};
+    if (__any(mb[384] != 0.0)) {
+      if (mb[384] != 0.0) {
+        if constexpr (ODOM_REGS) odometry_advance(odom[0], odom[1], odom[2], odom[3], P, ov.x, ov.y, ov.z, &odom_cache);
+        else odometry_step(rb, P, ov.x, ov.y, ov.z, &odom_cache);
+      }
+    }
+  };
+  constexpr int kWalkerThread = HELPER ? 128 : 0, kModelThread = HELPER ? 0 : 128;
   if (walker) {
     for (;;) {
       SHC_R2_ITER_BEGIN();
@@ -1131,7 +1220,35 @@
       }
       SHC_TICK(23);
       if (kind == IT_EXIT) break;
-      SHC_R2_ITER_END(0, 19, 20, 21, 2, 3, 4, 5, 6, 7, 16, 8, 17, 15, 29, 22, 23);
+      SHC_R2_ITER_END(kWalkerThread, 19, 20, 21, 2, 3, 4, 5, 6, 7, 16, 8, 17, 15, 29, 22, 23);
+      if (kind == IT_REAL) ++c_front;
+      prev_real = kind == IT_REAL;
+      __syncthreads();
+      ++k;
+    }
+  } else if (helper) {
+    if constexpr (HELPER) for (;;) {
+      SHC_R2_ITER_BEGIN();
+      const int kind = __builtin_amdgcn_readfirstlane(int(X.ctrl[k & 3][0]));
+      const u64 h0 = uni64(X.ctrl[k & 3][1]), h1 = uni64(X.ctrl[k & 3][2]);
+      SHC_TICK(29);
+      int nk = IT_EXIT;
+      u64 nh0v = 0, nh1v = 0;
+      if (leader && kind != IT_EXIT) leader_decide(kind, nk, nh0v, nh1v);
+      if (active) {
+        SHC_TICK(24);
+        if (kind == IT_REAL) pose_of_cycle(h0, h1);
+        SHC_TICK(25);
+        if (prev_real) {
+          if (FT::odom(P)) odometry_of_cycle(&X.mailbox[pair][c_back & 1][0][lane]);
+          ++c_back;
+        }
+        SHC_TICK(26);
+      }
+      if (leader && kind != IT_EXIT && lane == 0) leader_announce(nk, nh0v, nh1v);
+      SHC_TICK(14);
+      if (kind == IT_EXIT) break;
+      SHC_R2_ITER_END(256, 19, 29, 24, 30, 25, 26, 14);
       if (kind == IT_REAL) ++c_front;
       prev_real = kind == IT_REAL;
       __syncthreads();
@@ -1143,59 +1260,12 @@
       const int kind = __builtin_amdgcn_readfirstlane(int(X.ctrl[k & 3][0]));
       const u64 h0 = uni64(X.ctrl[k & 3][1]), h1 = uni64(X.ctrl[k & 3][2]);
       SHC_TICK(29);
-      int nk = IT_EXIT;
-      u64 nh0v = 0, nh1v = 0;
-      if (leader && kind != IT_EXIT) {
-        u64 gate;
-        if (kind == IT_BUBBLE) {
-          __builtin_amdgcn_s_sleep(2);
-          gate = uni64(ld_agent(&A.ctl->gate));
-        } else {
-          gate = uni64(gate_pref);
-        }
-        const unsigned db = unsigned(gate), sp = unsigned(gate >> 32);
-        const unsigned cn = c_front + (kind == IT_REAL ? 1u : 0u);
-        nk = cn >= sp ? IT_EXIT : (cn < db ? IT_REAL : IT_BUBBLE);
-        if (nk == IT_BUBBLE) {
-          const u64 now = wall_clock64();
-          if (bubble_since == 0) bubble_since = now;
-          else if (now - bubble_since > emergency_ticks) nk = IT_EXIT, held.fault = true;
-        } else {
-          bubble_since = 0;
-        }
-        if (nk == IT_REAL) {
-          const u64 *hp = reinterpret_cast<const u64 *>(A.headers + (cn & (kResidentHeaders - 1)));
-          nh0v = ld_agent(hp);
-          nh1v = ld_agent(hp + 1);
-        }
-        if (kind == IT_BUBBLE) gate_pref = gate;
-        else gate_pref = ld_agent(&A.ctl->gate);
-      }
+      [[maybe_unused]] int nk = IT_EXIT;
+      [[maybe_unused]] u64 nh0v = 0, nh1v = 0;
+      if constexpr (!HELPER) if (leader && kind != IT_EXIT) leader_decide(kind, nk, nh0v, nh1v);
       if (active) {
         SHC_TICK(24);
-        if constexpr (POSE_SPLIT) if (kind == IT_REAL) {
-          resident_take_inputs<RPW, ROBOT_POSE, false>(A, c_front, h0, h1, wave, lane, tile, tile_i, dirty, held, st.n_robots);
-          SHC_TICK(30);
-          double pose_c = -1.0;
-#pragma unroll
-          for (int j = 0; j < L; ++j) {
-            const double cj = X.pose_c[pair][c_front & 1][g.base + j];
-            pose_c = cj >= 0.0 ? cj : pose_c;
-          }
-          int lw[L] = {};
-          const double *mb = &X.mailbox[pair][c_front & 1][0][lane];
-          const V3 plane_prev{mb[7 * 64], mb[8 * 64], mb[9 * 64]}, pnorm_prev{mb[10 * 64], mb[11 * 64], mb[12 * 64]};
-          int rword_unused = 0;
-          Pose ap = pose_identity(), la = pose_identity();
-#ifdef SHC_ABLATE
-          if (!(P.debug_skip & 2048))
-#endif
-          (void)cycle_pose<L, NJ, F, true>(s, C, P, C.leg[leg], rb, g, leg, lw, rword_unused, 0, dirty, manual_live, ap, la, plane_prev, pnorm_prev, fb.uf.swing_c_count, 0,
-                                           &owpp_cache, &pose_c);
-          __builtin_amdgcn_fence(__ATOMIC_RELEASE, "workgroup");
-          __builtin_amdgcn_wave_barrier();
-          if (lane == 0) *const_cast<volatile unsigned *>(&X.pose_done[pair]) = c_front + 1;
-        }
+        if constexpr (POSE_SPLIT && !HELPER) if (kind == IT_REAL) pose_of_cycle(h0, h1);
         SHC_TICK(25);
         if (prev_real) {
           resident_take_inputs<RPW, ROBOT_NONE, true>(A, c_back, prev_h0, prev_h1, wave, lane, tile, tile_i, dirty, held, st.n_robots);
@@ -1208,15 +1278,7 @@
           SHC_TICK(31);
           const double *mb = &X.mailbox[pair][c_back & 1][0][lane];
           out.poser_tip = V3{mb[0], mb[64], mb[128]};
-          if constexpr (!ODOM_WALKER) if (FT::odom(P)) {
-            const V3 ov{mb[192], mb[256], mb[320]};
-            if (__any(mb[384] != 0.0)) {
-              if (mb[384] != 0.0) {
-                if constexpr (ODOM_REGS) odometry_advance(odom[0], odom[1], odom[2], odom[3], P, ov.x, ov.y, ov.z, &odom_cache);
-                else odometry_step(rb, P, ov.x, ov.y, ov.z, &odom_cache);
-              }
-            }
-          }
+          if constexpr (!ODOM_WALKER && !HELPER) if (FT::odom(P)) odometry_of_cycle(mb);
           out.adm_delta = V3{0, 0, 0};
           if (FT::adm(P)) cycle_admittance<NJ>(s, out, P, in);
           s.word = 0;
@@ -1253,14 +1315,10 @@
           if (lane == 0) st_agent(A.progress + wave, u64(c_back));
         }
       }
-      if (leader && kind != IT_EXIT && lane == 0) {
-        X.ctrl[(k + 1) & 3][0] = u64(nk);
-        X.ctrl[(k + 1) & 3][1] = nh0v;
-        X.ctrl[(k + 1) & 3][2] = nh1v;
-      }
+      if constexpr (!HELPER) if (leader && kind != IT_EXIT && lane == 0) leader_announce(nk, nh0v, nh1v);
       SHC_TICK(14);
       if (kind == IT_EXIT) break;
-      SHC_R2_ITER_END(128, 19, 29, 24, 30, 25, 31, 26, 9, 10, 11, 12, 27, 13, 28, 14);
+      SHC_R2_ITER_END(kModelThread, 19, 29, 24, 30, 25, 31, 26, 9, 10, 11, 12, 27, 13, 28, 14);
       if (kind == IT_REAL) ++c_front;
       prev_real = kind == IT_REAL;
       prev_h0 = h0, prev_h1 = h1;
@@ -1273,18 +1331,15 @@
 #undef SHC_R2_PHASES
 #ifdef SHC_RES2_TIMING
   if (blockIdx.x == 1 && lane == 0 && pair == 0) {
-    unsigned long long *dbg = reinterpret_cast<unsigned long long *>(A.ctl) + 8 + (walker ? 0 : 4);
+    unsigned long long *rec = reinterpret_cast<unsigned long long *>(A.ctl) + 8, *dbg = rec + (walker ? 0 : helper ? 72 : 4);
     dbg[0] = tm_busy, dbg[1] = tm_real, dbg[2] = __builtin_readcyclecounter() - tm_total0, dbg[3] = k;
 #ifndef SHC_RES2_BUSY_ONLY
-    if (walker) {
-      for (int i = 0; i < 32; ++i) dbg[8 + i] = (unsigned long long)shc_acc_lds[i];
-    } else {
-      for (int i = 0; i < 32; ++i) dbg[36 + i] = (unsigned long long)shc_acc_lds[32 + i];
-    }
+    const int from = int(threadIdx.x >> 7) * 32, to = walker ? 8 : helper ? 80 : 40;
+    for (int i = 0; i < 32; ++i) rec[to + i] = (unsigned long long)shc_acc_lds[from + i];
 #endif
   }
 #endif
-  if (active && ODOM_REGS && FT::odom(P) && walker == ODOM_WALKER) {
+  if (active && ODOM_REGS && FT::odom(P) && odom_mine) {
 #pragma unroll
     for (int i = 0; i < 4; ++i) rb.put(R::ODOM + i, odom[i]);
   }
@@ -1292,21 +1347,25 @@
     if (walker) {
       X.stiff[pair][lane] = s.stiff;
     } else {
-      X.ikfail[pair][lane] = s.word & LW_IKFAIL;
-      if (POSE_SPLIT) {
-        unsigned d = 0;
-#pragma unroll
-        for (unsigned b = 1; b <= DIRTY_LAST; b <<= 1)
-          if (__any((dirty & b) != 0)) d |= b;
-        if (lane == 0) X.model_dirty[pair] = d, X.model_seen[pair] = held.seen;
-      }
-      if (lane == 0) X.model_fault[pair] = held.fault ? 1u : 0u;
+      if (!helper) X.ikfail[pair][lane] = s.word & LW_IKFAIL;
+      if constexpr (HELPER) if (!helper && lane == 0) X.back_seen[pair] = held.seen;
+      if (poser) {
+        if (POSE_SPLIT) {
+          unsigned d = 0;
+#pragma unroll
+          for (unsigned b = 1; b <= DIRTY_LAST; b <<= 1)
+            if (__any((dirty & b) != 0)) d |= b;
+          if (lane == 0) X.model_dirty[pair] = d, X.model_seen[pair] = held.seen;
+        }
+        if (lane == 0) X.model_fault[pair] = held.fault ? 1u : 0u;
+      }
     }
   }
   __syncthreads();
-  if (!active) return;
+  if (!active || helper) return;
   if (walker) {
     if (POSE_SPLIT) dirty |= X.model_dirty[pair], held.seen |= X.model_seen[pair];
+    if constexpr (HELPER) held.seen |= X.back_seen[pair];
     if (X.model_fault[pair]) held.fault = true;
     if (c_front > 0) s.word = (s.word & ~LW_IKFAIL) | X.ikfail[pair][lane];
     {
diff --git a/syropod_highlevel_controller_amd/csrc/shc_cycle_launch.hpp b/syropod_highlevel_controller_amd/csrc/shc_cycle_launch.hpp
--- a/syropod_highlevel_controller_amd/csrc/shc_cycle_launch.hpp
+++ b/syropod_highlevel_controller_amd/csrc/shc_cycle_launch.hpp
@@ -18,7 +18,7 @@
   unsigned long long exited;
   unsigned long long fault;
   unsigned long long pad[5];
-  unsigned long long dbg[80];
+  unsigned long long dbg[112];
 };
 struct ResidentHost {
   unsigned long long doorbell;
@@ -81,6 +81,7 @@
   int supported;
   int blocks_per_cu;
   int two_wave;
+  int helper_wave;
   int batch;
 };
 
diff --git a/syropod_highlevel_controller_amd/csrc/shc_cycle_select.hpp b/syropod_highlevel_controller_amd/csrc/shc_cycle_select.hpp
--- a/syropod_highlevel_controller_amd/csrc/shc_cycle_select.hpp
+++ b/syropod_highlevel_controller_amd/csrc/shc_cycle_select.hpp
@@ -67,6 +67,7 @@
 constexpr bool has_resident(unsigned F) { return (F & F_MLEGS) == 0 && (SHC_GENERIC_LOOP_FORMS || (F & F_DYN) == 0 || (F & (F_TERRAIN | F_ROT)) == 0); }
 constexpr bool has_batch(unsigned F) { return (F & F_MLEGS) == 0 && (SHC_GENERIC_LOOP_FORMS || (F & F_DYN) == 0); }
 constexpr bool has_two_wave(unsigned F) { return has_resident(F) && (F & (F_TERRAIN | F_ROT)) == 0; }
+constexpr bool has_helper_wave(int L, int NJ, unsigned F) { return L == 6 && NJ == 3 && (F == F_C2 || F == (F_C2 | F_TIPF)); }
 constexpr bool has_half_kernels(unsigned F) { return (F & F_ROT) != 0 && (F & (F_DYN | F_TERRAIN | F_MLEGS | F_AUTO)) == 0; }
 
 }
diff --git a/syropod_highlevel_controller_amd/csrc/shc_resident.hpp b/syropod_highlevel_controller_amd/csrc/shc_resident.hpp
--- a/syropod_highlevel_controller_amd/csrc/shc_resident.hpp
+++ b/syropod_highlevel_controller_amd/csrc/shc_resident.hpp
@@ -29,6 +29,7 @@
   bool stream_doorbell_pending = false;
   unsigned groups_posted = 0;
   bool two_wave = false;
+  bool helper_wave = false;
   long long direct_last = -1;
 };
 
@@ -177,7 +178,7 @@
 }
 
 static int resident_fit(const shc_engine *e, ResidentFit &fit) {
-  fit = ResidentFit{0, 0, 0, 0};
+  fit = ResidentFit{};
   CycleLaunch a = cycle_launch(e);
   a.fit = &fit;
   return launch_cycle_for(e, a);
@@ -313,11 +314,13 @@
   e->plan_poser_tips_current = false;
   const bool two_wave = fit.two_wave && !(e->features & SHC_FEAT_RESIDENT_ONE_WAVE) && (e->n_waves + 1) / 2 + 1 <= prop.multiProcessorCount;
   r->two_wave = two_wave;
+  const char *two_role = getenv("SHC_RESIDENT_TWO_ROLE");
+  r->helper_wave = two_wave && fit.helper_wave && !(two_role && atoi(two_role) > 0);
   HIP_TRY(hipEventRecord(r->loop_ev, e->stream));
   HIP_TRY(hipStreamWaitEvent(r->loop_stream, r->loop_ev, 0));
   CycleLaunch a = cycle_launch(e);
   a.stream = r->loop_stream, a.resident = &A;
-  a.grid = two_wave ? unsigned((e->n_waves + 1) / 2 + 1) : unsigned(e->n_waves + 1), a.block = two_wave ? 256 : 64;
+  a.grid = two_wave ? unsigned((e->n_waves + 1) / 2 + 1) : unsigned(e->n_waves + 1), a.block = r->helper_wave ? 384 : two_wave ? 256 : 64;
   {
     const int rc = launch_cycle_for(e, a);
     if (rc != SHC_OK) return rc;
@@ -603,9 +606,11 @@
   if (err == hipSuccess) {
     ResidentCtl c;
     (void)hipMemcpy(&c, r->ctl, sizeof c, hipMemcpyDeviceToHost);
-    for (int w = 0; w < 2; ++w)
-      fprintf(stderr, "[res2 timing] %s: %.0f clocks busy per steady REAL iteration (%llu of them), loop %llu clocks, %llu iterations\n", w ? "model " : "walker",
-              c.dbg[4 * w + 1] ? double(c.dbg[4 * w]) / double(c.dbg[4 * w + 1]) : 0.0, c.dbg[4 * w + 1], c.dbg[4 * w + 2], c.dbg[4 * w + 3]);
+    for (int w = 0; w < (r->helper_wave ? 3 : 2); ++w) {
+      const unsigned long long *b = c.dbg + (w == 2 ? 72 : 4 * w);
+      fprintf(stderr, "[res2 timing] %s: %.0f clocks busy per steady REAL iteration (%llu of them), loop %llu clocks, %llu iterations\n", w == 0 ? "walker" : w == 1 ? "model " : "helper",
+              b[1] ? double(b[0]) / double(b[1]) : 0.0, b[1], b[2], b[3]);
+    }
 #ifndef SHC_RES2_BUSY_ONLY
     const int order[] = {20, 21, 2, 3, 4, 5, 6, 7, 16, 8, 17, 15, 29, 22, 23};
     const char *wname[] = {"control words (LDS) read", "inputs of the cycle taken", "cycle_front entry", "robot word / command read, stop predicates", "(pose elsewhere)", "getLimit",
@@ -621,7 +626,18 @@
                            "wait for the previous stores + progress word", "output-ring stores issued", "control words written (leader: waits for its loads)"};
     const double mits = c.dbg[5] ? double(c.dbg[5]) : 1.0;
     fprintf(stderr, "[res2 timing] model wavefront of pair 0 (the leader), mean clocks per phase:\n");
-    for (int i = 0; i < int(sizeof(morder) / sizeof(int)); ++i) fprintf(stderr, "[res2 timing]   model  t%-2d %-58s %7.0f\n", morder[i], mname[i], double(c.dbg[40 + morder[i]]) / mits);
+    for (int i = 0; i < int(sizeof(morder) / sizeof(int)); ++i) {
+      if (r->helper_wave && (morder[i] == 30 || morder[i] == 25)) continue;
+      fprintf(stderr, "[res2 timing]   model  t%-2d %-58s %7.0f\n", morder[i], mname[i], double(c.dbg[40 + morder[i]]) / mits);
+    }
+    if (r->helper_wave) {
+      const int horder[] = {29, 24, 30, 25, 26, 14};
+      const char *hname[] = {"control words (LDS) read", "leader: gate, what the next iteration is, header prefetch issued", "pose inputs of the cycle taken",
+                             "leg words reduced, updateCurrentPose of the walker's cycle + flag", "odometry", "control words written (leader: waits for its loads)"};
+      const double hits = c.dbg[73] ? double(c.dbg[73]) : 1.0;
+      fprintf(stderr, "[res2 timing] helper wavefront of pair 0 (the leader), mean clocks per phase:\n");
+      for (int i = 0; i < int(sizeof(horder) / sizeof(int)); ++i) fprintf(stderr, "[res2 timing]   helper t%-2d %-58s %7.0f\n", horder[i], hname[i], double(c.dbg[80 + horder[i]]) / hits);
+    }
 #endif
   }
 #endif
```
